# salute-developers/GigaAM

Hardware: AMD Instinct MI355X
Metric: RTFx v2_ctc batch32x20s (log-mel + encoder + greedy decode) (higher is better)
Workload: dtype f32 (GEMMs: 3-term split on fp16 MFMA, fp32 accumulate)

## Files before the change

### gigaam_amd/_lib.py

```python
from __future__ import annotations

import ctypes as C
import os
from typing import Optional

_HERE = os.path.dirname(os.path.abspath(__file__))
LIB_NAME = "libgigaam_hip.so"
LIB_PATH = os.path.join(_HERE, LIB_NAME)

SUBS_CONV2D, SUBS_CONV1D = 0, 1
ATT_ROTARY, ATT_REL_POS = 0, 1
NORM_BATCH, NORM_LAYER = 0, 1
HEAD_NONE, HEAD_CTC, HEAD_RNNT, HEAD_EMO = 0, 1, 2, 3
DTYPE_F32, DTYPE_F16, DTYPE_BF16, DTYPE_F64, DTYPE_I64 = 0, 1, 2, 3, 4
GEMM_F32, GEMM_F16X3, GEMM_F16 = 0, 1, 2
RS_U8, RS_I16, RS_I24, RS_I32, RS_F32, RS_MULAW, RS_ALAW = range(7)
RS_FORM_SINGLE, RS_FORM_TABLE, RS_FORM_ROWS = 0, 1, 2
PF_CLASSES = ["gemm", "conv2", "attn", "norm", "convmod", "stem", "frontend", "decode", "misc", "align_bt", "align_out"]


class GamConfig(C.Structure):
    _fields_ = [(n, C.c_int32) for n in (
        "sample_rate", "n_mels", "hop_length", "win_length", "n_fft", "center",
        "feat_in", "n_layers", "d_model", "subsampling", "subs_kernel_size", "subsampling_factor",
        "ff_expansion_factor", "self_attention_model", "n_heads", "pos_emb_max_len",
        "conv_norm_type", "conv_kernel_size",
        "head_type", "num_classes", "pred_hidden", "pred_rnn_layers", "joint_hidden",
    )]


_P = C.c_void_p


class GamLnOp(C.Structure):
    _fields_ = ([(n, _P) for n in ("x", "out1", "out2", "w1", "b1", "w2", "b2", "rcos", "rsin", "row_t", "rs", "part", "pbias", "presid",
                                   "xstore")]
                + [(n, C.c_int32) for n in ("mode", "rows", "d", "split1", "split2", "dk", "ta", "rope_rows", "nsplit")]
                + [("eps", C.c_float), ("palpha", C.c_float)])


SIGNATURES = {
    "gam_abi_version": (C.c_int, []),
    "gam_create": (C.c_int, [C.POINTER(GamConfig), C.c_int, C.POINTER(_P)]),
    "gam_destroy": (None, [_P]),
    "gam_set_weight": (C.c_int, [_P, C.c_char_p, _P, C.c_int, C.POINTER(C.c_int64), C.c_int]),
    "gam_finalize": (C.c_int, [_P]),
    "gam_feat_frames": (C.c_int64, [_P, C.c_int64]),
    "gam_enc_frames": (C.c_int64, [_P, C.c_int64]),
    "gam_frontend": (C.c_int, [_P, _P, _P, C.c_int, C.c_int64, _P, _P, _P]),
    "gam_encode": (C.c_int, [_P, _P, _P, C.c_int, C.c_int64, _P, _P, _P]),
    "gam_encode_ex": (C.c_int, [_P, _P, _P, C.c_int, C.c_int64, _P, _P, C.c_int, _P, _P]),
    "gam_encode_varlen": (C.c_int, [_P, _P, _P, C.POINTER(C.c_int64), C.c_int, C.c_int64, _P, _P, C.c_int, _P, _P]),
    "gam_last_encode_rows": (C.c_int, [_P, C.POINTER(C.c_int)]),
    "gam_ctc_head": (C.c_int, [_P, _P, C.c_int, C.c_int64, _P, _P]),
    "gam_ctc_greedy": (C.c_int, [_P, _P, _P, C.c_int, C.c_int64, _P, _P, _P, _P]),
    "gam_ctc_align": (C.c_int, [_P, _P, _P, C.c_int, C.c_int64, _P, _P, C.c_int, _P, _P, _P, _P, _P, _P, _P]),
    "gam_op_ctc_align": (C.c_int, [_P, _P, _P, C.c_int, C.c_int64, C.c_int, _P, _P, C.c_int, _P, _P, _P, _P, _P, _P, _P]),
    "gam_op_ctc_align_long": (C.c_int, [_P, _P, C.c_int64, C.c_int, _P, C.c_int, _P, _P, _P, _P, _P, _P, _P]),
    "gam_op_ctc_star_row": (C.c_int, [_P, _P, _P, C.c_int, C.c_int64, C.c_int, C.c_float, _P, _P]),
    "gam_ctc_align_star": (C.c_int, [_P, _P, _P, C.c_int, C.c_int64, _P, _P, C.c_int, C.c_float, _P, _P, _P, _P, _P, _P, _P]),
    "gam_op_ctc_align_star": (C.c_int, [_P, _P, _P, C.c_int, C.c_int64, C.c_int, _P, _P, _P, C.c_int, _P, _P, _P, _P, _P, _P, _P]),
    "gam_op_ctc_align_long_star": (C.c_int, [_P, _P, C.c_int64, C.c_int, _P, _P, C.c_int, _P, _P, _P, _P, _P, _P, _P]),
    "gam_op_ctc_stitch": (C.c_int, [_P, _P, _P, C.c_int, C.c_int64, C.c_int, _P, _P, _P, _P, C.c_int64, _P, _P]),
    "gam_op_ctc_greedy_long": (C.c_int, [_P, _P, C.c_int64, C.c_int, _P, _P, _P, _P]),
    "gam_set_ctc_align_workspace": (C.c_int, [_P, C.c_int64]),
    "gam_tune_ctc_align_long": (C.c_int, [C.c_int, C.c_int]),
    "gam_ctc_kws": (C.c_int, [_P, _P, _P, C.c_int, C.c_int64, C.c_int, _P, _P, _P, _P, _P, _P]),
    "gam_op_ctc_kws": (C.c_int, [_P, _P, _P, C.c_int, C.c_int64, C.c_int, C.c_int, _P, _P, _P, _P, _P, _P]),
    "gam_set_keywords": (C.c_int, [_P, _P, _P, C.c_int, _P]),
    "gam_ctc_kws_state_bytes": (C.c_int64, [_P]),
    "gam_op_ctc_kws_stream": (C.c_int, [_P, _P, C.c_int64, C.c_int, C.c_int64, C.c_int, _P, C.c_int, _P, _P, _P, _P, _P, _P, _P]),
    "gam_ctc_beam": (C.c_int, [_P, _P, _P, C.c_int, C.c_int64, C.c_int, _P, _P, _P, _P, _P, _P]),
    "gam_op_ctc_beam": (C.c_int, [_P, _P, _P, C.c_int, C.c_int64, C.c_int, C.c_int, _P, _P, _P, _P, _P, _P]),
    "gam_ctc_beam_stream_bytes": (C.c_int64, [_P, C.c_int, C.c_int64]),
    "gam_op_ctc_beam_stream": (C.c_int, [_P, _P, C.c_int64, C.c_int, C.c_int64, C.c_int, C.c_int, _P, C.c_int64, _P, _P, _P, _P, _P, _P, _P]),
    "gam_set_hotwords": (C.c_int, [_P, _P, _P, C.c_int, C.c_float]),
    "gam_set_lm": (C.c_int, [_P, _P, C.c_int, _P, C.c_int64, C.c_int, _P, C.c_int64, C.c_int, C.c_int, C.c_int, C.c_int, C.c_int,
                             C.c_float, C.c_float, C.c_float]),
    "gam_rnnt_greedy": (C.c_int, [_P, _P, _P, C.c_int, C.c_int64, C.c_int, _P, _P, _P, _P, _P, C.c_int, _P]),
    "gam_rnnt_encp": (C.c_int, [_P, _P, C.c_int, C.c_int64, _P, _P]),
    "gam_op_rnnt_greedy": (C.c_int, [_P, _P, _P, C.c_int, C.c_int64, C.c_int, _P, _P, _P, _P]),
    "gam_rnnt_greedy_stream_bytes": (C.c_int64, [_P]),
    "gam_op_rnnt_greedy_stream": (C.c_int, [_P, _P, C.c_int64, C.c_int64, C.c_int, C.c_int, _P, C.c_int64, _P, _P, C.c_int64, _P, _P, _P]),
    "gam_ctc_beam_nbest": (C.c_int, [_P, _P, _P, C.c_int, C.c_int64, C.c_int, C.c_int, _P, _P, _P, _P, _P, _P, _P]),
    "gam_op_ctc_beam_nbest": (C.c_int, [_P, _P, _P, C.c_int, C.c_int64, C.c_int, C.c_int, C.c_int, _P, _P, _P, _P, _P, _P, _P]),
    "gam_rnnt_beam_nbest": (C.c_int, [_P, _P, _P, C.c_int, C.c_int64, C.c_int, C.c_int, C.c_int, _P, _P, _P, _P, _P, _P, _P]),
    "gam_op_rnnt_beam_nbest": (C.c_int, [_P, _P, _P, C.c_int, C.c_int64, C.c_int, C.c_int, C.c_int, _P, _P, _P, _P, _P, _P, _P]),
    "gam_rnnt_beam": (C.c_int, [_P, _P, _P, C.c_int, C.c_int64, C.c_int, C.c_int, _P, _P, _P, _P, _P, _P]),
    "gam_op_rnnt_beam": (C.c_int, [_P, _P, _P, C.c_int, C.c_int64, C.c_int, C.c_int, _P, _P, _P, _P, _P, _P]),
    "gam_rnnt_align": (C.c_int, [_P, _P, _P, C.c_int, C.c_int64, _P, _P, C.c_int, _P, _P, _P, _P, _P]),
    "gam_op_rnnt_align": (C.c_int, [_P, _P, _P, C.c_int, C.c_int64, _P, _P, C.c_int, _P, _P, _P, _P, _P, _P]),
    "gam_op_rnnt_lattice_align": (C.c_int, [_P, _P, _P, C.c_int, C.c_int64, C.c_int, _P, _P, C.c_int, _P, _P, _P, _P, _P]),
    "gam_set_rnnt_align_workspace": (C.c_int, [_P, C.c_int64]),
    "gam_ctc_confidence": (C.c_int, [_P, _P, _P, C.c_int, C.c_int64, _P, _P, _P, C.c_int, C.c_int, C.c_int, _P, _P, _P, _P]),
    "gam_op_ctc_confidence": (C.c_int, [_P, _P, _P, C.c_int, C.c_int64, C.c_int, _P, _P, _P, C.c_int, C.c_int, C.c_int, _P, _P, _P, _P]),
    "gam_op_ctc_confidence_long": (C.c_int, [_P, _P, C.c_int64, C.c_int, _P, _P, _P, C.c_int, C.c_int, C.c_int, C.c_int, _P, _P, _P, _P]),
    "gam_rnnt_confidence": (C.c_int, [_P, _P, _P, C.c_int, C.c_int64, _P, _P, _P, C.c_int, C.c_int, _P, _P, _P]),
    "gam_op_rnnt_confidence": (C.c_int, [_P, _P, _P, C.c_int, C.c_int64, _P, _P, _P, C.c_int, C.c_int, _P, _P, _P]),
    "gam_emo_probs": (C.c_int, [_P, _P, _P, C.c_int, C.c_int64, _P, _P]),
    "gam_rnnt_predict": (C.c_int, [_P, _P, _P, _P, C.c_int, _P, _P, _P, _P]),
    "gam_rnnt_joint": (C.c_int, [_P, _P, _P, C.c_int, C.c_int, C.c_int, _P, _P]),
    "gam_set_gemm_mode": (C.c_int, [_P, C.c_int]),
    "gam_get_gemm_mode": (C.c_int, [_P]),
    "gam_set_rnnt_cluster": (C.c_int, [_P, C.c_int]),
    "gam_get_rnnt_cluster": (C.c_int, [_P]),
    "gam_rnnt_cluster_plan_info": (C.c_int, [C.c_int] * 8 + [C.POINTER(C.c_int32)]),
    "gam_rnnt_last_decode": (C.c_int, [_P, C.POINTER(C.c_int32)]),
    "gam_debug_buffer_hash": (C.c_int, [_P, C.c_int, C.POINTER(C.c_uint64), C.POINTER(C.c_int64)]),
    "gam_range_flag": (C.c_int, [_P, C.POINTER(C.c_int), _P]),
    "gam_range_flag_fetch": (C.c_int, [_P, _P, _P]),
    "gam_op_gemm": (C.c_int, [_P, _P, _P, _P, _P, C.c_int, C.c_int, C.c_int, C.c_int, _P]),
    "gam_op_gemm_ex": (C.c_int, [_P, _P, _P, _P, _P, C.c_float, _P, C.c_int, C.c_int, C.c_int, C.c_int, _P]),
    "gam_op_gemm_fmt": (C.c_int, [_P, _P, _P, _P, _P, C.c_float, _P, C.c_int64, C.c_int, C.c_int, C.c_int, C.c_int, C.c_int, C.c_int, _P]),
    "gam_op_attention": (C.c_int, [_P, _P, _P, _P, _P, _P, C.c_int, C.c_int, C.c_int, _P]),
    "gam_op_attention_ex": (C.c_int, [_P, _P, _P, _P, C.c_int64, _P, _P, _P, C.c_int, C.c_int, C.c_int, C.c_int, _P, _P, _P, _P]),
    "gam_op_layernorm": (C.c_int, [_P, C.POINTER(GamLnOp), _P]),
    "gam_op_convmod": (C.c_int, [_P, _P, _P, _P, _P, _P, _P, _P, _P, C.c_int, C.c_int, C.c_int, C.c_int, C.c_int, C.c_int, C.c_int, _P]),
    "gam_tune_sp": (C.c_int, [C.c_int, C.c_int, C.c_int]),
    "gam_plan_sp": (C.c_int, [C.c_int, C.c_int, C.c_int, C.c_int, C.POINTER(C.c_int), C.POINTER(C.c_int), C.POINTER(C.c_int)]),
    "gam_plan_sp_ex": (C.c_int, [C.c_int, C.c_int, C.c_int, C.c_int, C.POINTER(C.c_int), C.POINTER(C.c_int), C.POINTER(C.c_int), C.POINTER(C.c_int)]),
    "gam_tune_sp_stages": (C.c_int, [C.c_int]),
    "gam_resample_plan": (C.c_int, [C.c_int, C.c_int, C.POINTER(C.c_int), C.POINTER(C.c_int), C.POINTER(C.c_int)]),
    "gam_resample_tile": (C.c_int, [C.c_int, C.c_int, C.POINTER(C.c_int), C.POINTER(C.c_int)]),
    "gam_resample_table": (C.c_int, [C.c_int, C.c_int, _P, _P]),
    "gam_resample_out_len": (C.c_int64, [C.c_int, C.c_int, C.c_int64]),
    "gam_op_resample": (C.c_int, [_P, C.c_int, C.c_int, C.c_int, _P, C.c_int, C.c_int64, C.c_int, C.c_int, _P, _P, _P, C.c_int64, _P, _P]),
    "gam_profile_enable": (C.c_int, [_P, C.c_int]),
    "gam_profile_pause": (C.c_int, [_P, C.c_int]),
    "gam_profile_read": (C.c_int, [_P, C.c_int, C.POINTER(C.c_double), C.POINTER(C.c_int64), C.POINTER(C.c_double)]),
    "gam_profile_read_bytes": (C.c_int, [_P, C.c_int, C.POINTER(C.c_double)]),
    "gam_last_error": (C.c_char_p, [_P]),
    "gam_comm_unique_id": (C.c_int, [C.c_char_p]),
    "gam_comm_create": (C.c_int, [C.c_char_p, C.c_int, C.c_int, C.c_int, C.POINTER(_P)]),
    "gam_comm_world": (C.c_int, [_P]),
    "gam_gather_ids": (C.c_int, [_P, _P, _P, _P, _P, C.c_int, C.c_int, _P, _P, _P, _P, _P]),
    "gam_comm_last_error": (C.c_char_p, [_P]),
    "gam_comm_destroy": (None, [_P]),
}

_lib: Optional[C.CDLL] = None


class GigaAMHipError(RuntimeError):
    pass


def load_library(path: Optional[str] = None) -> C.CDLL:
    global _lib
    if _lib is not None and path is None:
        return _lib
    p = path or os.environ.get("GIGAAM_HIP_LIB", LIB_PATH)
    if not os.path.exists(p):
        raise GigaAMHipError(
            f"{p} not found: the HIP extension is not built. Run `python -c 'import __graft_entry__ as g; g.build()'` "
            "(hipcc --offload-arch=gfx950). There is no CPU fallback.")
    lib = C.CDLL(p)
    for name, (res, args) in SIGNATURES.items():
        fn = getattr(lib, name)
        fn.restype = res
        fn.argtypes = args
    if lib.gam_abi_version() != 1:
        raise GigaAMHipError("libgigaam_hip.so ABI version mismatch")
    if path is None:
        _lib = lib
    return lib
```

### gigaam_amd/csrc/gam_api.hip

```cpp
#include <hip/hip_runtime.h>

#include <algorithm>
#include <cmath>
#include <cstdarg>
#include <cstdio>
#include <cstring>
#include <map>
#include <string>
#include <vector>

#include "../../include/gigaam_hip.h"
#include "gam_align.h"
#include "gam_align_long.h"
#include "gam_kws.h"
#include "gam_attn.h"
#include "gam_beam.h"
#include "gam_beam_stream.h"
#include "gam_rnnt_beam.h"
#include "gam_attn16.h"
#include "gam_comm.h"
#include "gam_common.h"
#include "gam_convmod.h"
#include "gam_decode.h"
#include "gam_rnnt_stream.h"
// ... 215 lines not shown
    if (x < 0x33000000u) return (uint16_t)sign;
    const int e = (int)(x >> 23);
    uint32_t m = (x & 0x7fffffu) | 0x800000u;
    const int shift = 126 - e;
    const uint32_t rem = m & ((1u << shift) - 1u), half = 1u << (shift - 1);
    m >>= shift;
    if (rem > half || (rem == half && (m & 1u))) ++m;
    return (uint16_t)(sign | m);
  }
  const uint32_t e = (x >> 23) - 112u;
  uint32_t m = x & 0x7fffffu;
  uint32_t h = (e << 10) | (m >> 13);
  const uint32_t rem = m & 0x1fffu;
  if (rem > 0x1000u || (rem == 0x1000u && (h & 1u))) ++h;
  return (uint16_t)(sign | h);
}

float half_to_float(uint16_t x) {
  const uint32_t sign = (x >> 15) & 1, exp = (x >> 10) & 0x1f, man = x & 0x3ff;
  uint32_t f;
  if (exp == 0) {
    if (man == 0) f = sign << 31;
    else {
      int e = -1; uint32_t m = man;
      do { ++e; m <<= 1; } while (!(m & 0x400));
      f = (sign << 31) | ((uint32_t)(127 - 15 - e) << 23) | ((m & 0x3ff) << 13);
    }
  } else if (exp == 31) f = (sign << 31) | 0x7f800000u | (man << 13);
  else f = (sign << 31) | ((exp + 127 - 15) << 23) | (man << 13);
  float r; memcpy(&r, &f, 4); return r;
}

int make_split(gam_handle* h, const std::vector<float>& w, W16& out, int K = 0, int conv_taps = 0) {
  float mx = 0.f;
  for (float v : w) mx = std::max(mx, fabsf(v));
  int shift = 0;
  if (mx > 0.f && std::isfinite(mx)) shift = (int)floorf(log2f(256.0f / mx));
  shift = std::max(-24, std::min(24, shift));
  const float sc = ldexpf(1.0f, shift);
  std::vector<uint16_t> hi(w.size()), lo(w.size());
  for (size_t i = 0; i < w.size(); ++i) {
    const float v = w[i] * sc;
    const uint16_t hb = float_to_half_bits(v);
    hi[i] = hb;
    lo[i] = float_to_half_bits(v - half_to_float(hb));
  }
  out.inv = ldexpf(1.0f, -shift);
  std::vector<uint16_t> hp(hi);
  if (conv_taps > 0 && K > 0 && (K / conv_taps) % 64 == 0 && w.size() % (size_t)K == 0) {
    const size_t C = (size_t)K / conv_taps, cb64 = C / 64;
    for (size_t n = 0; n < w.size() / K; ++n)
      for (size_t cb = 0; cb < cb64; ++cb)
        for (size_t t = 0; t < (size_t)conv_taps; ++t)
          for (size_t j = 0; j < 64; ++j)
            hp[n * K + (cb * conv_taps + t) * 64 + j] = hi[n * K + t * C + cb * 64 + j];
  }
  out.h16 = (_Float16*)dev_upload(h, hp.data(), w.size() * 2, std::max<size_t>(w.size(), 8) * 2 + 64);
  if (!out.h16) return -2;
  if (K > 0 && K % 32 == 0 && w.size() % (size_t)K == 0) {
    std::vector<uint16_t> sp(w.size() * 2);
    for (size_t i = 0; i < w.size(); ++i) {
      const size_t n = i / K, k = i % K;
      size_t kb = k / 32;
      if (conv_taps > 0) {
        const size_t cblocks = (size_t)K / conv_taps / 32, t = kb / cblocks, cb = kb % cblocks;
        kb = cb * conv_taps + t;
      }
      const size_t o = n * 2 * (size_t)K + kb * 64 + (k % 32);
      sp[o] = hi[i];
      sp[o + 32] = lo[i];
    }
    out.sp = (_Float16*)dev_upload(h, sp.data(), sp.size() * 2, sp.size() * 2 + 64);
    if (!out.sp) return -2;
  }
  return 0;
}

const HostTensor* find(gam_handle* h, const std::string& key) {
  auto it = h->staged.find(key);
  return it == h->staged.end() ? nullptr : &it->second;
}

struct ProfScope {
  gam_handle* h;
  hipStream_t s;
  ProfEvent* ev = nullptr;
  ProfScope(gam_handle* h_, hipStream_t s_, int cls, double work) : h(h_), s(s_) {
    if (!h->prof_on || (h->prof_on == 2 && cls != GAM_PF_GEMM && cls != GAM_PF_CONV2)) return;
    if (h->prof_used == h->prof_events.size()) {
      ProfEvent e;
      if (hipEventCreate(&e.a) != hipSuccess || hipEventCreate(&e.b) != hipSuccess) return;
      h->prof_events.push_back(e);
    }
    ev = &h->prof_events[h->prof_used++];
    ev->cls = cls;
    h->prof_work[cls] += work;
    h->prof_launches[cls] += 1;
    hipEventRecord(ev->a, s);
  }
  ~ProfScope() {
    if (ev) hipEventRecord(ev->b, s);
  }
};

struct PendingReduce {
  const float* part = nullptr;
  int nsplit = 0;
  const float* bias = nullptr;
  const float* resid = nullptr;
  float alpha = 1.0f;
  GamGemmArgs full;
  int act = 0;
  void clear() { part = nullptr; nsplit = 0; }
};

int flush_pending(gam_handle* h, hipStream_t s, PendingReduce* p) {
  if (p == nullptr || p->part == nullptr) return 0;
  const hipError_t e = gam_launch_splitk_reduce(p->full, p->act, p->nsplit, s);
  const int M = p->full.M, N = p->full.N;
  p->clear();
  if (e != hipSuccess) return fail(h, -2, "split-K reduce launch (M=%d N=%d): %s", M, N, hipGetErrorString(e));
  return 0;
}

static inline bool split_mode(const gam_handle* h) { return h->gemm_mode != GAM_GEMM_F32; }

int gemm(gam_handle* h, hipStream_t s, const GamGemmArgs& a_in, int act, int cls = GAM_PF_GEMM, const W16* w16 = nullptr,
         PendingReduce* defer = nullptr) {
  GamGemmArgs a = a_in;
  if (int r = flush_pending(h, s, defer)) return r;
  a.range_flag = h->use_range ? h->range_flag : nullptr;
  if (!split_mode(h)) a.c_guard = 0;
  ProfScope ps(h, s, cls, 2.0 * (double)a.M * (double)a.N * (double)a.K);
  if (ps.ev) {
    const double abytes = a.a_mode == 0 ? ((double)(a.M - 1) * (double)std::min<long>(a.lda, a.K) + a.K) * 4.0
                                        : (double)a.M / a.conv_f2 * 2.0 * a.conv_fp * a.conv_c * 4.0;
    h->prof_bytes[cls] += abytes * (a.n_switch > 0 ? 2.0 : 1.0) + 4.0 * a.N * a.K + 4.0 * a.M * a.N * (a.R ? 2.0 : 1.0);
  }
  hipError_t e;
  if (a.Asp != nullptr) {
    if (!split_mode(h)) return fail(h, -2, "sp32 A operand outside the split-fp16 GEMM mode");
    if (w16 == nullptr || w16->sp == nullptr) return fail(h, -2, "sp32 A without sp32 W planes");
    a.wscale_inv = w16->inv;
    a.Wsp = w16->sp;
    a.h16 = 0;
    if (a.a_fmt == 2) {
      if (a.K % 64 != 0 || (a.a_mode == 0 ? a.lda % 64 != 0 : a.conv_c % 64 != 0) || w16->h16 == nullptr)
        return fail(h, -2, "GAM_GEMM_F16: K / row pitch of a GEMM operand is not a multiple of 64 (M=%d N=%d K=%d)", a.M, a.N, a.K);
      a.h16 = 1; a.K /= 2; a.lda /= 2; a.conv_c /= 2;
      a.Wsp = w16->h16;
    }
    GamSpPlan plan = gam_gemm_sp_plan(a.M, a.N, a.K, a.a_mode, h->ncu);
    if (!h->use_splitk) plan.s = 1;
    a.sp_mt = plan.mt; a.sp_nw = plan.nw; a.sp_ns = plan.ns;
    GamGemmArgs full = a;
    if (plan.s > 1) {
      if (int r = ensure(h, h->splitk_ws, (size_t)plan.s * a.M * a.N + 64)) return r;
      a.splitk = plan.s; a.partial = h->splitk_ws.p;
    }
    e = gam_launch_gemm_sp(a, act, s);
    if (e != hipSuccess) return fail(h, -2, "sp gemm launch (M=%d N=%d K=%d): %s", a.M, a.N, a.K, hipGetErrorString(e));
    if (plan.s > 1 && defer != nullptr && h->fuse_reduce && act == GAM_ACT_NONE && !a.c_split && !a.c_guard && a.lens == nullptr &&
        !a.remap && a.ldc == a.N && a.bias != nullptr && a.R != nullptr && a.ldr == a.N) {
      defer->part = a.partial; defer->nsplit = plan.s; defer->bias = a.bias; defer->resid = a.R; defer->alpha = a.alpha;
      defer->full = full; defer->full.partial = a.partial; defer->act = act;
    } else if (plan.s > 1) {
      full.partial = a.partial;
      e = gam_launch_splitk_reduce(full, act, plan.s, s);
      if (e != hipSuccess) return fail(h, -2, "split-K reduce launch (M=%d N=%d): %s", a.M, a.N, hipGetErrorString(e));
    }
    return 0;
  }
  if (a.a_rs != nullptr || a.c_split) return fail(h, -2, "row-scaled A or split C without sp32 operands (M=%d N=%d K=%d)", a.M, a.N, a.K);
  int S = 1;
  if (h->use_splitk && a.a_mode == 0 && a.K % 32 == 0) {
    const int tiles = gam_cdiv(a.M, 128) * gam_cdiv(a.N, 128), nk = a.K / 32, ncu = 256;
    if (tiles * 2 <= ncu && nk >= 4) {
      S = std::min(16, std::min(ncu / tiles, nk / 2));
      while (S > 1 && nk % S != 0) --S;
    }
  }
  GamGemmArgs full = a;
  if (S > 1) {
    DevBuf& ws = cls == GAM_PF_DECODE ? h->dec_splitk_ws : h->splitk_ws;
    if (int r = ensure(h, ws, (size_t)S * a.M * a.N + 64)) return r;
    a.splitk = S; a.ldw = a.K; a.K = a.K / S; a.partial = ws.p;
  }
  e = gam_launch_gemm(a, act, s);
  if (e != hipSuccess) return fail(h, -2, "gemm launch (M=%d N=%d K=%d): %s", a.M, a.N, a.K, hipGetErrorString(e));
  if (S > 1) {
    full.partial = a.partial;
    e = gam_launch_splitk_reduce(full, act, S, s);
    if (e != hipSuccess) return fail(h, -2, "split-K reduce launch (M=%d N=%d): %s", a.M, a.N, hipGetErrorString(e));
  }
  return 0;
}

GamGemmArgs gemm_args(const float* A, long lda, const float* W, const float* bias, float* C, long ldc, int M, int N, int K) {
  GamGemmArgs g;
  memset(&g, 0, sizeof g);
  g.A = A; g.W = W; g.bias = bias; g.C = C; g.R = nullptr;
  g.M = M; g.N = N; g.K = K; g.lda = lda; g.ldc = ldc; g.ldr = ldc; g.alpha = 1.0f;
  g.rpb = 1; g.fdiv = 1;
  return g;
}

int layernorm(gam_handle* h, hipStream_t s, GamLnArgs a, int mode, PendingReduce* pend = nullptr) {
  if (pend != nullptr && pend->part != nullptr) {
    const GamGemmArgs& g = pend->full;
    if (a.x == g.C && a.rows == g.M && a.d == g.N && g.ldc == g.N) {
      a.part = pend->part; a.nsplit = pend->nsplit; a.pbias = pend->bias; a.presid = pend->resid; a.palpha = pend->alpha;
      a.xstore = const_cast<float*>(a.x);
      pend->clear();
    } else if (int r = flush_pending(h, s, pend)) {
      return r;
    }
  }
  const double bytes = (double)a.rows * a.d * 4.0 * (mode == 0 ? 2.0 : 3.0);
  ProfScope ps(h, s, GAM_PF_NORM, bytes);
  hipError_t e = gam_launch_layernorm(a, mode, s);
  if (e != hipSuccess) return fail(h, -2, "layernorm launch: %s", hipGetErrorString(e));
  return 0;
}

int64_t half_up(int64_t l) { return l <= 0 ? 0 : (l + 1) / 2; }

struct DecodeScope {
  gam_handle* h;
  hipStream_t s;
  DecodeScope(gam_handle* h_, hipStream_t s_) : h(h_), s(s_) {
    if (h->dec_evt == nullptr && hipEventCreateWithFlags(&h->dec_evt, hipEventDisableTiming) != hipSuccess) { h->dec_evt = nullptr; (void)hipGetLastError(); }
    if (h->dec_evt != nullptr && h->dec_evt_set && h->dec_stream != s) (void)hipStreamWaitEvent(s, h->dec_evt, 0);
  }
  ~DecodeScope() {
    if (h->dec_evt != nullptr && hipEventRecord(h->dec_evt, s) == hipSuccess) { h->dec_stream = s; h->dec_evt_set = true; }
  }
};

#define GAM_DECODE_ENTRY(h, stream)      \
  hipStream_t s = (hipStream_t)(stream); \
  if (!(h)) return -1;                   \
  HIPCHK(h, hipSetDevice((h)->device));  \
  DecodeScope ds(h, s)

int head_check(gam_handle* h, int want, const char* who) {
  if (!h) return -1;
  if (who && !h->finalized) return fail(h, -1, "%s before gam_finalize", who);
  if (h->cfg.head_type != want || !h->has_head)
    return fail(h, -1, "model has no %s head", want == GAM_HEAD_CTC ? "CTC" : want == GAM_HEAD_RNNT ? "RNN-T" : "emotion");
  return 0;
}

template <class Args> void rnnt_pred_weights(const gam_handle* h, Args& a) {
  a.gate_tab = h->lstm_tab; a.whh_t = h->lstm_whh_t; a.wih_x = h->lstm_wih_x; a.whh_x = h->lstm_whh_x; a.bias_x = h->lstm_bias_x;
}
template <class Args> void rnnt_joint_weights(const gam_handle* h, Args& a) {
  a.wpred_t = h->jn_pred_t; a.bpred = h->jn_pred_b; a.wout = h->jn_out_w; a.bout = h->jn_out_b;
}

}

extern "C" {

int gam_abi_version(void) { return GAM_ABI_VERSION; }

const char* gam_last_error(const gam_handle* h) { return h ? h->err.c_str() : "null handle"; }

int gam_create(const gam_config* cfg, int device_id, gam_handle** out) {
  if (!cfg || !out) return -1;
  gam_handle* h = new gam_handle();
  h->cfg = *cfg;
  h->device = device_id;
  *out = h;
  if (const char* e = getenv("GAM_SPLITK")) h->use_splitk = atoi(e);
  if (const char* e = getenv("GAM_PACK")) h->use_pack = atoi(e);
  if (const char* e = getenv("GAM_FUSE_REDUCE")) h->fuse_reduce = atoi(e);
  if (const char* e = getenv("GAM_GRAPH")) h->use_graph = atoi(e);
  if (const char* e = getenv("GAM_GRAPH_MAX_ROWS")) h->graph_max_rows = atoi(e);
  if (const char* e = getenv("GAM_RNNT_CLUSTER")) h->rnnt_cluster = std::max(-1, std::min(8, atoi(e)));
  if (const char* e = getenv("GAM_RNNT_ALIGN_WS")) h->ra_ws_limit = (size_t)std::max(1ll, atoll(e));
  if (const char* e = getenv("GAM_CTC_ALIGN_WS")) h->al_ws_limit = (size_t)std::max(1ll, atoll(e));
  if (const char* e = getenv("GAM_RNNT_EXCLUSIVE")) h->rnnt_exclusive = atoi(e);
  if (const char* e = getenv("GAM_RNNT_COOP")) h->rnnt_coop = atoi(e);
  if (const char* e = getenv("GAM_RNNT_FORCE_TIMEOUT")) h->rnnt_force_timeout = atoi(e);
  if (const char* e = getenv("GAM_RNNT_NO_REPAIR")) h->rnnt_no_repair = atoi(e);
  {
    int n = 0;
    if (hipDeviceGetAttribute(&n, hipDeviceAttributeMultiprocessorCount, device_id) == hipSuccess && n > 0) h->ncu = n;
    int co = 0;
    if (hipDeviceGetAttribute(&co, hipDeviceAttributeCooperativeLaunch, device_id) != hipSuccess || co == 0) h->rnnt_coop = 0;
  }
  if (const char* e = getenv("GAM_ROWSCALE")) h->use_rowscale = atoi(e);
  if (const char* e = getenv("GAM_RANGE")) h->use_range = atoi(e);
  if (const char* e = getenv("GAM_GEMM_MODE"))
    h->gemm_mode = strcmp(e, "f32") == 0 ? GAM_GEMM_F32 : (strcmp(e, "f16") == 0 ? GAM_GEMM_F16 : GAM_GEMM_F16X3);
  const gam_config& c = h->cfg;
  if (c.d_model <= 0 || c.n_heads <= 0 || c.d_model % c.n_heads != 0)
    return fail(h, -1, "bad d_model/n_heads %d/%d", c.d_model, c.n_heads);
  if (c.d_model / c.n_heads != GAM_ATT_DK) return fail(h, -1, "head dim %d unsupported (kernels are built for %d)", c.d_model / c.n_heads, GAM_ATT_DK);
  if (c.d_model % 64 != 0 || c.d_model > 1024) return fail(h, -1, "d_model %d unsupported", c.d_model);
  if (c.subsampling_factor != 4) return fail(h, -1, "subsampling_factor %d unsupported", c.subsampling_factor);
  if (c.subsampling == GAM_SUBS_CONV2D && c.subs_kernel_size != 3) return fail(h, -1, "conv2d stem needs kernel 3");
  if (c.subsampling == GAM_SUBS_CONV1D && c.subs_kernel_size != 5) return fail(h, -1, "conv1d stem needs kernel 5");
  if (c.win_length != c.n_fft) return fail(h, -1, "win_length != n_fft unsupported");
  if (c.n_mels > 64 || c.n_mels != c.feat_in) return fail(h, -1, "n_mels %d / feat_in %d unsupported", c.n_mels, c.feat_in);
  if (c.head_type == GAM_HEAD_RNNT && (c.pred_rnn_layers < 1 || c.pred_rnn_layers > 4 || c.pred_hidden > GAM_RNNT_MAXH || c.joint_hidden > GAM_RNNT_MAXH || c.num_classes > GAM_RNNT_MAXV || c.joint_hidden % 16 != 0 || c.pred_hidden % 16 != 0))
    return fail(h, -1, "RNN-T head shape unsupported");
// ... 623 lines not shown

static int enc_stem(gam_handle* h, hipStream_t s, const EncPlan& p, const EncBufs& w, const float* feat) {
  if (int r = p.conv2d ? stem_conv2d(h, s, p, w, feat) : stem_conv1d(h, s, p, w, feat)) return r;
  if (p.packed) {
    ProfScope ps(h, s, GAM_PF_STEM, (double)p.NR * p.D * 8.0);
    hipLaunchKernelGGL(gam_gather_rows_kernel, dim3(std::min(4096, gam_cdiv(p.NR * (p.D / 4), 256))), dim3(256), 0, s, h->y.p, w.row_src, h->x.p, p.NR, p.D);
    HIPCHK(h, hipGetLastError());
  }
  return 0;
}

static int launch_attention(gam_handle* h, hipStream_t s, const float* q, const float* k, const float* v, long ldq, float* ctx, int ctx_split,
                            const int* lens, const int* cu, int B, int Ta, int Tv, int H, const float* pbuf, const float* pos_u,
                            const float* pos_v) {
  const int D = H * GAM_ATT_DK;
  GamAttnArgs at;
  memset(&at, 0, sizeof at);
  at.q = q; at.k = k; at.v = v; at.ctx = ctx; at.ctx_split = ctx_split; at.lens = lens; at.cu = cu;
  at.B = B; at.Ta = Ta; at.Tv = Tv; at.H = H; at.ldq = ldq; at.ldv = ldq; at.ldo = D;
  at.scale = 1.0f / sqrtf((float)GAM_ATT_DK);
  at.pbuf = pbuf; at.pos_u = pos_u; at.pos_v = pos_v; at.ldp = D;
  hipError_t e = gam_launch_attn_mode(at, GAM_ATT_DK, split_mode(h), s, h->gemm_mode == GAM_GEMM_F16 ? 1 : 3, h->ncu);
  if (e != hipSuccess) return fail(h, -2, "attention launch: %s", hipGetErrorString(e));
  return 0;
}

static hipError_t launch_convmod(gam_handle* h, hipStream_t s, const float* u, float* z, const float* dw_w, const float* dw_b, const float* n_scale,
                                 const float* n_shift, const int* lens, const int* cu, int B, int Ta, int Tv, int d, int ks, bool layer_norm,
                                 int z_split) {
  GamConvModArgs cm;
  memset(&cm, 0, sizeof cm);
  cm.u = u; cm.z = z; cm.dw_w = dw_w; cm.dw_b = dw_b; cm.n_scale = n_scale; cm.n_shift = n_shift;
  cm.lens = lens; cm.cu = cu; cm.B = B; cm.Ta = Ta; cm.Tv = Tv; cm.d = d; cm.ks = ks; cm.eps = 1e-5f;
  cm.z_split = z_split; cm.range_flag = h->use_range ? h->range_flag : nullptr;
  return gam_launch_convmod(cm, layer_norm, s);
}

static int norm_to_y(gam_handle* h, hipStream_t s, const EncCtx& c, const float* w, const float* b, PendingReduce* pend) {
  GamLnArgs a = c.ln;
  a.x = h->x.p; a.out1 = h->y.p; a.w1 = w; a.b1 = b;
  a.split1 = c.p.spf;
  return layernorm(h, s, a, 0, pend);
}

static int ffn_block(gam_handle* h, hipStream_t s, const EncCtx& c, const float* w1, const float* b1, const W16& s_w1, const float* w2,
                     const float* b2, const W16& s_w2, PendingReduce* pend) {
  const int D = c.p.D, DFF = c.p.DFF, NR = c.p.NR, spf = c.p.spf;
  GamGemmArgs g = gemm_args(h->y.p, D, w1, b1, h->hbuf.p, DFF, NR, DFF, D);
  gemm_formats(g, spf, c.w.rs, spf, 1);
  if (int r = gemm(h, s, g, GAM_ACT_SILU, GAM_PF_GEMM, &s_w1)) return r;
  GamGemmArgs g2 = gemm_args(h->hbuf.p, DFF, w2, b2, h->x.p, D, NR, D, DFF);
  g2.R = h->x.p; g2.ldr = D; g2.alpha = 0.5f;
  gemm_formats(g2, spf, nullptr, 0, 0);
  return gemm(h, s, g2, GAM_ACT_NONE, GAM_PF_GEMM, &s_w2, pend);
}

static int attn_block(gam_handle* h, hipStream_t s, const EncCtx& c, const LayerW& L, PendingReduce* pend) {
  const EncPlan& p = c.p;
  const int D = p.D, NR = p.NR, Tv = p.Tv, spf = p.spf;
  float* const rs = c.w.rs;
  GamLnArgs a = c.ln;
  a.x = h->x.p; a.out1 = h->y.p; a.out2 = h->yr.p; a.w1 = L.ln_att_w; a.b1 = L.ln_att_b;
  a.split1 = spf; a.split2 = spf;
  if (int r = layernorm(h, s, a, p.rel ? 0 : 1, pend)) return r;
  const bool one_launch = p.rel || (p.sp && (2 * D) % 256 == 0);
  if (one_launch) {
    GamGemmArgs gq = gemm_args(p.rel ? h->y.p : h->yr.p, D, L.wqkv, L.bqkv, h->qkv.p, 3 * D, NR, 3 * D, D);
    gemm_formats(gq, spf, rs, 0, 1);
    if (!p.rel) { gq.Asp2 = reinterpret_cast<const _Float16*>(h->y.p); gq.n_switch = 2 * D; }
    if (int r = gemm(h, s, gq, GAM_ACT_NONE, GAM_PF_GEMM, &L.s_wqkv)) return r;
  } else {
    GamGemmArgs gq = gemm_args(h->yr.p, D, L.wqkv, L.bqkv, h->qkv.p, 3 * D, NR, 2 * D, D);
    gemm_formats(gq, spf, rs, 0, 1);
    if (int r = gemm(h, s, gq, GAM_ACT_NONE, GAM_PF_GEMM, &L.s_wqkv)) return r;
    W16 wv16 = L.s_wqkv;
    const size_t off = (size_t)2 * D * D;
    wv16.h16 += off;
    if (wv16.sp) wv16.sp += 2 * off;
    GamGemmArgs gv = gemm_args(h->y.p, D, L.wqkv + off, L.bqkv + 2 * D, h->qkv.p + 2 * D, 3 * D, NR, D, D);
    gemm_formats(gv, spf, rs, 0, 1);
    if (int r = gemm(h, s, gv, GAM_ACT_NONE, GAM_PF_GEMM, &wv16)) return r;
  }
  if (p.rel) {
    const size_t pe0 = (size_t)(h->cfg.pos_emb_max_len - 1 - (Tv - 1)) * D;
    GamGemmArgs gp = gemm_args(h->rel_pe + pe0, D, L.wpos, nullptr, h->pbuf.p, D, 2 * Tv - 1, D, D);
    if (p.sp) { gp.Asp = reinterpret_cast<const _Float16*>(h->rel_pe_sp + pe0); gp.a_fmt = 1; }
    if (int r = gemm(h, s, gp, GAM_ACT_NONE, GAM_PF_GEMM, &L.s_wpos)) return r;
  }
  {
    ProfScope ps(h, s, GAM_PF_ATTN, 4.0 * (double)p.B * p.H * (double)Tv * Tv * p.dk);
    if (int r = launch_attention(h, s, h->qkv.p, h->qkv.p + D, h->qkv.p + 2 * D, 3 * D, h->ctx.p, spf, p.B > 1 ? c.w.len2 : nullptr, c.w.cu, p.B,
                                 p.packed ? p.Tmax : p.Ta, Tv, p.H, p.rel ? h->pbuf.p : nullptr, L.pos_u, L.pos_v))
      return r;
  }
  GamGemmArgs go = gemm_args(h->ctx.p, D, L.wo, L.bo, h->x.p, D, NR, D, D);
  go.R = h->x.p; go.ldr = D;
  gemm_formats(go, spf, nullptr, 0, 0);
  return gemm(h, s, go, GAM_ACT_NONE, GAM_PF_GEMM, &L.s_wo, pend);
}

static int conv_block(gam_handle* h, hipStream_t s, const EncCtx& c, const LayerW& L, PendingReduce* pend) {
  const EncPlan& p = c.p;
  const int D = p.D, NR = p.NR, ks = h->cfg.conv_kernel_size;
  if (int r = norm_to_y(h, s, c, L.ln_conv_w, L.ln_conv_b, pend)) return r;
  GamGemmArgs g1 = gemm_args(h->y.p, D, L.pw1_w, L.pw1_b, h->ubuf.p, 2 * D, NR, 2 * D, D);
  gemm_formats(g1, p.spf, c.w.rs, 0, 0);
  if (int r = gemm(h, s, g1, GAM_ACT_NONE, GAM_PF_GEMM, &L.s_pw1)) return r;
  {
    ProfScope ps(h, s, GAM_PF_CONVMOD, (double)NR * D * 3 * 4.0);
    hipError_t e = launch_convmod(h, s, h->ubuf.p, h->zbuf.p, L.dw_w, L.dw_b, L.cn_scale, L.cn_shift, c.w.len2, c.w.cu, p.B,
                                  p.packed ? p.Tmax : p.Ta, p.Tv, D, ks, h->cfg.conv_norm_type == GAM_NORM_LAYER, p.spf);
    if (e != hipSuccess) return fail(h, -2, "conv-module launch (k=%d): %s", ks, hipGetErrorString(e));
  }
  GamGemmArgs g2 = gemm_args(h->zbuf.p, D, L.pw2_w, L.pw2_b, h->x.p, D, NR, D, D);
  g2.R = h->x.p; g2.ldr = D;
  gemm_formats(g2, p.spf, nullptr, 0, 0);
  return gemm(h, s, g2, GAM_ACT_NONE, GAM_PF_GEMM, &L.s_pw2, pend);
}

static int norm_out_block(gam_handle* h, hipStream_t s, const EncCtx& c, const LayerW& L, const LayerW* next, PendingReduce* pend) {
  GamLnArgs a = c.ln;
  a.x = h->x.p; a.out1 = h->x.p; a.w1 = L.ln_out_w; a.b1 = L.ln_out_b;
  if (next != nullptr) {
    a.out2 = h->y.p; a.w2 = next->ln_ff1_w; a.b2 = next->ln_ff1_b;
    a.split2 = c.p.spf;
    return layernorm(h, s, a, 2, pend);
  }
  a.rs = nullptr;
  return layernorm(h, s, a, 0, pend);
}

static int run_layers(gam_handle* h, hipStream_t s, const EncCtx& c) {
  const int nl = c.p.nl;
  if (nl > 0)
    if (int r = norm_to_y(h, s, c, h->layers[0].ln_ff1_w, h->layers[0].ln_ff1_b, nullptr)) return r;
  PendingReduce pend;
  for (int li = 0; li < nl; ++li) {
    const LayerW& L = h->layers[li];
    if (int r = ffn_block(h, s, c, L.ff1_w1, L.ff1_b1, L.s_ff1_w1, L.ff1_w2, L.ff1_b2, L.s_ff1_w2, &pend)) return r;
    if (int r = attn_block(h, s, c, L, &pend)) return r;
    if (int r = conv_block(h, s, c, L, &pend)) return r;
    if (int r = norm_to_y(h, s, c, L.ln_ff2_w, L.ln_ff2_b, &pend)) return r;
    if (int r = ffn_block(h, s, c, L.ff2_w1, L.ff2_b1, L.s_ff2_w1, L.ff2_w2, L.ff2_b2, L.s_ff2_w2, &pend)) return r;
    if (int r = norm_out_block(h, s, c, L, li + 1 < nl ? &h->layers[li + 1] : nullptr, &pend)) return r;
  }
  return flush_pending(h, s, &pend);
}

static int replay_layers(gam_handle* h, hipStream_t s, const EncCtx& c, bool* replayed) {
  typedef gam_handle::GraphEntry Entry;
  const EncPlan& p = c.p;
  *replayed = false;
  if (!p.graph) return 0;
  const GamSpForce& frc = gam_sp_force();
  const std::vector<int> key = {p.B, p.Ta, p.Tv, p.nl, h->gemm_mode, (int)p.sp, h->use_splitk, h->fuse_reduce, frc.mt.load(), frc.nw.load(), frc.s.load(), frc.ns.load()};
  Entry& ge = h->graphs[key];
  if (ge.gen != h->ws_generation) {
    if (ge.exec) { hipGraphExecDestroy(ge.exec); --h->graph_count; }
    ge = Entry();
    ge.gen = h->ws_generation;
  }
  if (ge.exec == nullptr && ge.seen == Entry::SEEN_ONCE && h->graph_count >= 32) ge.seen = Entry::PLAIN_ONLY;
  if (ge.exec == nullptr && ge.seen == Entry::SEEN_ONCE) {
    hipGraph_t graph = nullptr;
    if (h->cap_stream == nullptr && hipStreamCreateWithFlags(&h->cap_stream, hipStreamNonBlocking) != hipSuccess)
      h->cap_stream = nullptr;
    if (h->cap_stream != nullptr && hipStreamBeginCapture(h->cap_stream, hipStreamCaptureModeRelaxed) == hipSuccess) {
      const int r = run_layers(h, h->cap_stream, c);
      const hipError_t e = hipStreamEndCapture(h->cap_stream, &graph);
      if (r == 0 && e == hipSuccess && graph != nullptr && h->ws_generation == ge.gen &&
          hipGraphInstantiate(&ge.exec, graph, nullptr, nullptr, 0) != hipSuccess)
        ge.exec = nullptr;
      if (graph) hipGraphDestroy(graph);
    }
    (void)hipGetLastError();
    if (ge.exec == nullptr) { ge.seen = Entry::PLAIN_ONLY; ++h->graph_captures_failed; }
    else ++h->graph_count;
  }
  if (ge.exec != nullptr) {
    HIPCHK(h, hipGraphLaunch(ge.exec, s));
    *replayed = true;
    ++h->graph_replays;
  } else if (ge.seen == Entry::UNSEEN) {
    ge.seen = Entry::SEEN_ONCE;
  }
  return 0;
}

static int enc_outputs(gam_handle* h, hipStream_t s, const EncPlan& p, const EncBufs& w, float* encoded, float* tokens_out, int32_t* enc_len) {
  const int B = p.B, Ta = p.Ta, Tv = p.Tv, D = p.D;
  ProfScope ps(h, s, GAM_PF_MISC, (double)B * Tv * D * 8.0);
  if (encoded && p.packed) {
    hipLaunchKernelGGL(gam_unpack_transpose_kernel, dim3(gam_cdiv(D, 32), gam_cdiv(Tv, 32), B), dim3(256), 0, s, h->x.p, w.cu, w.len2, encoded, Tv, D);
    HIPCHK(h, hipGetLastError());
  } else if (encoded) {
    hipError_t e = gam_launch_transpose(h->x.p, encoded, B, Tv, D, (size_t)Ta * D, D, (size_t)D * Tv, Tv, s);
    if (e != hipSuccess) return fail(h, -2, "transpose launch: %s", hipGetErrorString(e));
  }
  if (tokens_out && p.packed) {
    hipLaunchKernelGGL(gam_unpack_rows_kernel, dim3(std::min(4096, gam_cdiv(B * Tv * (D / 4), 256))), dim3(256), 0, s, h->x.p, w.cu, w.len2, tokens_out, B, Tv, D);
    HIPCHK(h, hipGetLastError());
  } else if (tokens_out)
    HIPCHK(h, hipMemcpy2DAsync(tokens_out, (size_t)Tv * D * 4, h->x.p, (size_t)Ta * D * 4, (size_t)Tv * D * 4, B, hipMemcpyDeviceToDevice, s));
  if (enc_len) HIPCHK(h, hipMemcpyAsync(enc_len, w.elen, (size_t)B * sizeof(int), hipMemcpyDeviceToDevice, s));
  return 0;
}

static int encode_impl(gam_handle* h, const float* feat, const int64_t* feat_len, int B, int64_t T, float* encoded,
                       int32_t* enc_len, int n_layers_run, float* tokens_out, hipStream_t s, const int64_t* feat_len_host = nullptr) {
  if (!h || !h->finalized) return fail(h, -1, "gam_encode before gam_finalize");
  if (!h->has_encoder) return fail(h, -1, "this handle was finalized without encoder weights");
  EncCtx c;
  if (int r = enc_plan(h, B, T, n_layers_run, feat_len_host, c.p)) return r;
  HIPCHK(h, hipSetDevice(h->device));
  h->last_rows = c.p.NR;
  h->last_rows_padded = c.p.N;
  if (int r = enc_workspace(h, c.p, c.w)) return r;
  c.ln = enc_ln_args(h, c.p, c.w);
  if (int r = enc_lengths(h, s, c.p, c.w, feat_len)) return r;
  if (int r = enc_stem(h, s, c.p, c.w, feat)) return r;
  bool replayed = false;
  if (int r = replay_layers(h, s, c, &replayed)) return r;
  if (!replayed)
    if (int r = run_layers(h, s, c)) return r;
  return enc_outputs(h, s, c.p, c.w, encoded, tokens_out, enc_len);
}

int gam_encode(gam_handle* h, const float* feat, const int64_t* feat_len, int B, int64_t T, float* encoded, int32_t* enc_len,
               void* stream) {
  return encode_impl(h, feat, feat_len, B, T, encoded, enc_len, -1, nullptr, (hipStream_t)stream);
}

int gam_encode_ex(gam_handle* h, const float* feat, const int64_t* feat_len, int B, int64_t T, float* encoded, int32_t* enc_len,
                  int n_layers_run, float* tokens_out, void* stream) {
  return encode_impl(h, feat, feat_len, B, T, encoded, enc_len, n_layers_run, tokens_out, (hipStream_t)stream);
}

int gam_encode_varlen(gam_handle* h, const float* feat, const int64_t* feat_len, const int64_t* feat_len_host, int B, int64_t T,
                      float* encoded, int32_t* enc_len, int n_layers_run, float* tokens_out, void* stream) {
  return encode_impl(h, feat, feat_len, B, T, encoded, enc_len, n_layers_run, tokens_out, (hipStream_t)stream, feat_len_host);
}

static int to_tokens(gam_handle* h, const float* encoded, int B, int64_t Tp, hipStream_t s) {
  const int D = h->cfg.d_model;
  if (int r = ensure(h, h->tok, (size_t)B * Tp * D)) return r;
  ProfScope ps(h, s, GAM_PF_DECODE, (double)B * Tp * D * 8.0);
  hipError_t e = gam_launch_transpose(encoded, h->tok.p, B, D, (int)Tp, (size_t)D * Tp, Tp, (size_t)Tp * D, D, s);
  if (e != hipSuccess) return fail(h, -2, "transpose launch: %s", hipGetErrorString(e));
  return 0;
}

static int ctc_logits(gam_handle* h, const float* encoded, int B, int64_t Tp, hipStream_t s) {
  if (B <= 0 || Tp <= 0) return fail(h, -1, "bad shape B=%d T'=%lld", B, (long long)Tp);
  HIPCHK(h, hipSetDevice(h->device));
  const int D = h->cfg.d_model, V = h->cfg.num_classes;
  if (int r = to_tokens(h, encoded, B, Tp, s)) return r;
  if (int r = ensure(h, h->logits, (size_t)B * Tp * V)) return r;
  GamGemmArgs g = gemm_args(h->tok.p, D, h->ctc_w, h->ctc_b, h->logits.p, V, (int)(B * Tp), V, D);
  return gemm(h, s, g, GAM_ACT_NONE, GAM_PF_DECODE);
}

static int rnnt_encp(gam_handle* h, const float* encoded, int B, int64_t Tp, hipStream_t s, float* out = nullptr) {
  const int D = h->cfg.d_model, JH = h->cfg.joint_hidden;
  if (int r = to_tokens(h, encoded, B, Tp, s)) return r;
  if (!out)
    if (int r = ensure(h, h->encp, (size_t)B * Tp * JH)) return r;
  GamGemmArgs g = gemm_args(h->tok.p, D, h->jn_enc_w, h->jn_enc_b, out ? out : h->encp.p, JH, (int)(B * Tp), JH, D);
  return gemm(h, s, g, GAM_ACT_NONE, GAM_PF_DECODE);
}

static int ctc_log_probs(gam_handle* h, const float* encoded, int B, int64_t Tp, float* out, hipStream_t s) {
  if (int r = ctc_logits(h, encoded, B, Tp, s)) return r;
  const int V = h->cfg.num_classes, rows = (int)(B * Tp);
  ProfScope ps(h, s, GAM_PF_DECODE, (double)rows * V * 8.0);
  hipLaunchKernelGGL(gam_log_softmax_kernel, dim3(gam_cdiv(rows, 4)), dim3(256), 0, s, h->logits.p, out ? out : h->logits.p, rows, V);
  HIPCHK(h, hipGetLastError());
  return 0;
}

int gam_ctc_head(gam_handle* h, const float* encoded, int B, int64_t Tp, float* log_probs, void* stream) {
  if (int r = head_check(h, GAM_HEAD_CTC, "CTC head")) return r;
  GAM_DECODE_ENTRY(h, stream);
  return ctc_log_probs(h, encoded, B, Tp, log_probs, s);
}

int gam_ctc_greedy(gam_handle* h, const float* encoded, const int32_t* enc_len, int B, int64_t Tp, int32_t* ids,
                   int32_t* frames, int32_t* counts, void* stream) {
  if (int r = head_check(h, GAM_HEAD_CTC, "CTC head")) return r;
  GAM_DECODE_ENTRY(h, stream);
  if (int r = ctc_logits(h, encoded, B, Tp, s)) return r;
  const int V = h->cfg.num_classes;
  const size_t sm = ((size_t)Tp + GAM_CTC_NT / 64 + 8) * sizeof(int);
  if (sm > 60 * 1024) return fail(h, -1, "T'=%lld too long for the CTC greedy kernel", (long long)Tp);
  ProfScope ps(h, s, GAM_PF_DECODE, (double)B * Tp * V * 4.0);
  hipLaunchKernelGGL(gam_ctc_greedy_kernel, dim3(B), dim3(GAM_CTC_NT), sm, s, h->logits.p, enc_len, (int)Tp, V, ids, frames, counts);
  HIPCHK(h, hipGetLastError());
  return 0;
}

static int ctc_align_launch(gam_handle* h, const float* lp, const int32_t* enc_len, int B, int64_t Tp, int V, const int32_t* targets,
                            const int32_t* target_len, int Umax, int32_t* frame_labels, int32_t* tok_first, int32_t* tok_last,
                            float* score, float* loglik, int32_t* status, hipStream_t s, const float* star = nullptr) {
  if (B <= 0 || Tp <= 0 || V < 2) return fail(h, -1, "CTC alignment: bad shape B=%d T'=%lld V=%d", B, (long long)Tp, V);
  if (Tp > GAM_ALIGN_MAX_T) return fail(h, -1, "CTC alignment: T'=%lld frames exceed the limit %d", (long long)Tp, GAM_ALIGN_MAX_T);
  if (Umax < 0 || Umax > GAM_ALIGN_MAX_U) return fail(h, -1, "CTC alignment: Umax=%d tokens outside [0, %d]", Umax, GAM_ALIGN_MAX_U);
  if (!lp || !enc_len || !target_len || !frame_labels || !score || !loglik || !status ||
      (Umax > 0 && (!targets || !tok_first || !tok_last)))
    return fail(h, -1, "CTC alignment: NULL buffer");
// ... 1327 lines not shown
  return launch_attention(h, (hipStream_t)stream, q, k, v, (long)ldq, ctx, 0, lens, cu, B, Ta, Tv, H, pbuf, pos_u, pos_v);
}

int gam_op_layernorm(gam_handle* h, const gam_ln_op* op, void* stream) {
  if (!h) return -1;
  if (!op) return fail(h, -1, "layernorm: null argument block");
  const gam_ln_op& o = *op;
  if (o.mode < 0 || o.mode > 2) return fail(h, -1, "layernorm: mode %d outside 0..2", o.mode);
  if (o.rows <= 0 || o.d <= 0) return fail(h, -1, "layernorm: bad shape rows %d d %d", o.rows, o.d);
  if (o.split1 < 0 || o.split1 > 2 || o.split2 < 0 || o.split2 > 2)
    return fail(h, -1, "layernorm: store format %d / %d outside 0..2", o.split1, o.split2);
  if (!o.out1 || !o.w1 || !o.b1) return fail(h, -1, "layernorm: out1 / w1 / b1 are mandatory");
  if (!o.part && !o.x) return fail(h, -1, "layernorm: x is mandatory without part");
  if (o.part && o.mode != 2 && !o.xstore) return fail(h, -1, "layernorm: part without xstore");
  if (o.mode != 0 && !o.out2) return fail(h, -1, "layernorm: mode %d needs out2", o.mode);
  if (o.mode == 2 && (!o.w2 || !o.b2)) return fail(h, -1, "layernorm: mode 2 needs w2 / b2");
  if (o.mode == 1) {
    if (!o.rcos || !o.rsin || o.rope_rows <= 0) return fail(h, -1, "layernorm: mode 1 needs rcos / rsin of rope_rows > 0 rows");
    if (o.dk <= 0) return fail(h, -1, "layernorm: mode 1 needs dk > 0");
    if (!o.row_t && o.ta <= 0) return fail(h, -1, "layernorm: mode 1 needs row_t or ta > 0");
  }
  auto al16 = [](const void* p) { return (reinterpret_cast<uintptr_t>(p) & 15) == 0; };
  if (!al16(o.x) || !al16(o.out1) || !al16(o.out2) || !al16(o.w1) || !al16(o.b1) || !al16(o.w2) || !al16(o.b2) || !al16(o.rcos) ||
      !al16(o.rsin) || !al16(o.part) || !al16(o.pbias) || !al16(o.presid) || !al16(o.xstore))
    return fail(h, -1, "layernorm: operands must be 16-byte aligned");
  HIPCHK(h, hipSetDevice(h->device));
  GamLnArgs a;
  memset(&a, 0, sizeof a);
  a.x = o.x; a.out1 = o.out1; a.out2 = o.out2; a.w1 = o.w1; a.b1 = o.b1; a.w2 = o.w2; a.b2 = o.b2;
  a.rcos = o.rcos; a.rsin = o.rsin; a.rows = o.rows; a.d = o.d; a.ta = o.ta; a.dk = o.dk; a.eps = o.eps;
  a.split1 = o.split1; a.split2 = o.split2; a.rs = o.rs; a.rope_rows = o.rope_rows;
  a.part = o.part; a.nsplit = o.nsplit; a.pbias = o.pbias; a.presid = o.presid; a.palpha = o.palpha; a.xstore = o.xstore;
  a.row_t = o.row_t;
  hipError_t e = gam_launch_layernorm(a, o.mode, (hipStream_t)stream);
  if (e != hipSuccess)
    return fail(h, -2, "layernorm launch (mode %d, rows %d, d %d, dk %d, split %d/%d, nsplit %d): %s", o.mode, o.rows, o.d, o.dk,
                o.split1, o.split2, o.part ? o.nsplit : 0, hipGetErrorString(e));
  return 0;
}

int gam_op_convmod(gam_handle* h, const float* u, float* z, const float* dw_w, const float* dw_b, const float* n_scale,
                   const float* n_shift, const int32_t* lens, const int32_t* cu, int B, int Ta, int Tv, int d, int ks, int layer_norm,
                   int z_split, void* stream) {
  if (!h) return -1;
  if (!h->finalized) return fail(h, -1, "gam_op_convmod before gam_finalize");
  if (!u || !z || !dw_w || !dw_b || !n_scale || !n_shift || !lens) return fail(h, -1, "conv module: null operand");
  if (B <= 0 || Ta <= 0 || Tv <= 0 || d <= 0) return fail(h, -1, "conv module: bad shape B %d Ta %d Tv %d d %d", B, Ta, Tv, d);
  if (cu == nullptr && Tv > Ta) return fail(h, -1, "conv module: Tv %d > Ta %d in the padded layout", Tv, Ta);
  if (z_split < 0 || z_split > 2) return fail(h, -1, "conv module: store format %d outside 0..2", z_split);
  if (z_split && d % 32 != 0) return fail(h, -1, "conv module: a split-fp16 z needs d %% 32 == 0 (d = %d)", d);
  auto al16 = [](const void* p) { return (reinterpret_cast<uintptr_t>(p) & 15) == 0; };
  if (d % 4 == 0 && (!al16(u) || !al16(z) || !al16(dw_b) || !al16(n_scale) || !al16(n_shift)))
    return fail(h, -1, "conv module: operands must be 16-byte aligned");
  HIPCHK(h, hipSetDevice(h->device));
  hipError_t e = launch_convmod(h, (hipStream_t)stream, u, z, dw_w, dw_b, n_scale, n_shift, lens, cu, B, Ta, Tv, d, ks, layer_norm != 0, z_split);
  if (e != hipSuccess) return fail(h, -2, "conv-module launch (k=%d, d=%d, %s): %s", ks, d, layer_norm ? "LayerNorm" : "BatchNorm", hipGetErrorString(e));
  return 0;
}

int gam_set_gemm_mode(gam_handle* h, int mode) {
  if (!h || (mode != GAM_GEMM_F32 && mode != GAM_GEMM_F16X3 && mode != GAM_GEMM_F16)) return fail(h, -1, "unknown GEMM mode %d", mode);
  h->gemm_mode = mode;
  return 0;
}

int gam_get_gemm_mode(const gam_handle* h) { return h ? h->gemm_mode : -1; }

int gam_debug_buffer_hash(gam_handle* h, int which, uint64_t* hash_out, int64_t* floats_out) {
  if (!h || !hash_out) return -1;
  const DevBuf* b = which == 0 ? &h->tok : which == 1 ? &h->encp : which == 2 ? &h->rnnt_x : which == 3 ? &h->logits : nullptr;
  if (!b) return fail(h, -1, "no such buffer %d", which);
  HIPCHK(h, hipSetDevice(h->device));
  HIPCHK(h, hipDeviceSynchronize());
  std::vector<uint32_t> host(b->cap);
  if (b->cap) HIPCHK(h, hipMemcpy(host.data(), b->p, b->cap * sizeof(float), hipMemcpyDeviceToHost));
  uint64_t x = 1469598103934665603ull;
  for (uint32_t v : host) { x ^= v; x *= 1099511628211ull; }
  *hash_out = x;
  if (floats_out) *floats_out = (int64_t)b->cap;
  return 0;
}

int gam_set_rnnt_cluster(gam_handle* h, int workgroups_per_utterance) {
  if (!h) return -1;
  if (workgroups_per_utterance < -1 || workgroups_per_utterance > 8) return fail(h, -1, "cluster size %d outside -1 (auto) .. 8", workgroups_per_utterance);
  h->rnnt_cluster = workgroups_per_utterance;
  return 0;
}

int gam_get_rnnt_cluster(gam_handle* h) { return h ? h->rnnt_cluster : -2; }

int gam_rnnt_cluster_plan_info(int ncu, int cluster, int exclusive, int B, int H, int JH, int V, int L, int32_t* out) {
  if (!out || B <= 0 || H <= 0 || JH <= 0 || V <= 0 || L <= 0) return -1;
  const RnntClusterPlan p = rnnt_cluster_plan(ncu, cluster, exclusive, B, H, JH, V, L);
  memset(out, 0, 8 * sizeof(int32_t));
  if (p.C == 0) return 0;
  out[0] = p.C; out[1] = p.nr; out[2] = p.kern; out[3] = p.resident ? 1 : 0;
  out[4] = p.wout_slice_in_lds; out[5] = p.wpred_slice_in_lds; out[6] = (int32_t)p.lds; out[7] = (int32_t)p.grid;
  return 0;
}

int gam_rnnt_last_decode(gam_handle* h, int32_t* out) {
  if (!h || !out) return -1;
  out[0] = h->last_rnnt_c; out[1] = h->last_rnnt_kern; out[2] = h->last_rnnt_refused;
  return 0;
}

int gam_last_encode_rows(gam_handle* h, int* rows_padded) {
  if (!h) return -1;
  if (rows_padded) *rows_padded = h->last_rows_padded;
  return h->last_rows;
}

int gam_range_flag(gam_handle* h, int* flag_host, void* stream) {
  if (!h || !flag_host) return -1;
  if (!h->finalized) return fail(h, -1, "gam_range_flag before gam_finalize");
  HIPCHK(h, hipSetDevice(h->device));
  hipStream_t s = (hipStream_t)stream;
  HIPCHK(h, hipMemcpyAsync(flag_host, h->range_flag, sizeof(int), hipMemcpyDeviceToHost, s));
  HIPCHK(h, hipMemsetAsync(h->range_flag, 0, sizeof(int), s));
  HIPCHK(h, hipStreamSynchronize(s));
  return 0;
}

int gam_range_flag_fetch(gam_handle* h, int32_t* flag_dev, void* stream) {
  if (!h || !flag_dev) return -1;
  if (!h->finalized) return fail(h, -1, "gam_range_flag_fetch before gam_finalize");
  HIPCHK(h, hipSetDevice(h->device));
  hipStream_t s = (hipStream_t)stream;
  HIPCHK(h, hipMemcpyAsync(flag_dev, h->range_flag, sizeof(int), hipMemcpyDeviceToDevice, s));
  HIPCHK(h, hipMemsetAsync(h->range_flag, 0, sizeof(int), s));
  return 0;
}

int gam_plan_sp(int M, int N, int K, int n_cu, int* mt, int* nw, int* splitk) {
  if (M <= 0 || N <= 0 || K <= 0 || K % 32 != 0 || !mt || !nw || !splitk) return -1;
  const GamSpPlan p = gam_gemm_sp_plan(M, N, K, 0, n_cu > 0 ? n_cu : 256);
  *mt = p.mt; *nw = p.nw; *splitk = p.s;
  return 0;
}

int gam_tune_sp(int mt, int nw, int splitk) {
  GamSpForce& f = gam_sp_force();
  f.mt = mt; f.nw = nw; f.s = splitk;
  return 0;
}

int gam_tune_sp_stages(int stages) {
  if (stages != 0 && stages != 2 && stages != 3) return -1;
  gam_sp_force().ns = stages;
  return 0;
}

int gam_plan_sp_ex(int M, int N, int K, int n_cu, int* mt, int* nw, int* splitk, int* stages) {
  if (M <= 0 || N <= 0 || K <= 0 || K % 32 != 0 || !mt || !nw || !splitk || !stages) return -1;
  const GamSpPlan p = gam_gemm_sp_plan(M, N, K, 0, n_cu > 0 ? n_cu : 256);
  *mt = p.mt; *nw = p.nw; *splitk = p.s; *stages = p.ns;
  return 0;
}

int gam_resample_plan(int rate_in, int rate_out, int* up, int* down, int* taps) {
  GamRsPlan p;
  const int rc = gam_rs_plan(rate_in, rate_out, &p);
  if (rc != 0) return rc;
  if (up) *up = (int)p.N;
  if (down) *down = (int)p.O;
  if (taps) *taps = p.K;
  return 0;
}

int gam_resample_tile(int rate_in, int rate_out, int* tile, int* form) {
  GamRsPlan p;
  const int rc = gam_rs_plan(rate_in, rate_out, &p);
  if (rc != 0) return rc;
  if (tile) *tile = p.tile;
  if (form) *form = p.form;
  return 0;
}

int gam_resample_table(int rate_in, int rate_out, float* coeff, int32_t* first) {
  GamRsPlan p;
  const int rc = gam_rs_plan(rate_in, rate_out, &p);
  if (rc != 0) return rc;
  if (!coeff || !first) return -1;
  gam_rs_table(p, coeff, first);
  return 0;
}

int64_t gam_resample_out_len(int rate_in, int rate_out, int64_t n_in) {
  GamRsPlan p;
  if (gam_rs_plan(rate_in, rate_out, &p) != 0) return -1;
  return gam_rs_out_len(p, n_in);
}

int gam_op_resample(const void* src, int fmt, int channels, int channel, const int64_t* len_in, int B, int64_t frames, int rate_in, int rate_out,
                    const float* coeff, const int32_t* first, float* dst, int64_t L_out, int64_t* len_out, void* stream) {
  return gam_rs_run(src, fmt, channels, channel, len_in, B, frames, rate_in, rate_out, coeff, first, dst, L_out, len_out, (hipStream_t)stream);
}

int gam_profile_enable(gam_handle* h, int on) {
  if (!h) return -1;
  h->prof_on = on;
  h->prof_used = 0;
  for (int i = 0; i < GAM_PF_NCLASS; ++i) { h->prof_work[i] = 0; h->prof_launches[i] = 0; h->prof_bytes[i] = 0; }
  return 0;
}

int gam_profile_pause(gam_handle* h, int on) {
  if (!h) return -1;
  h->prof_on = on;
  return 0;
}

int gam_profile_read_bytes(gam_handle* h, int cls, double* bytes) {
  if (!h || cls < 0 || cls >= GAM_PF_NCLASS || !bytes) return -1;
  *bytes = h->prof_bytes[cls];
  return 0;
}

int gam_profile_read(gam_handle* h, int cls, double* ms, int64_t* launches, double* work) {
  if (!h || cls < 0 || cls >= GAM_PF_NCLASS) return -1;
  double tot = 0;
  for (size_t i = 0; i < h->prof_used; ++i) {
    ProfEvent& e = h->prof_events[i];
    if (e.cls != cls) continue;
    HIPCHK(h, hipEventSynchronize(e.b));
    float t = 0;
    HIPCHK(h, hipEventElapsedTime(&t, e.a, e.b));
    tot += t;
  }
  if (ms) *ms = tot;
  if (launches) *launches = h->prof_launches[cls];
  if (work) *work = h->prof_work[cls];
  return 0;
}

}
```

### gigaam_amd/csrc/gam_gemm.h

```cpp
#pragma once
#include "gam_common.h"
#include <stdlib.h>

struct GamGemmArgs {
  const float* A;
  const float* W;
  const float* bias;
  const float* R;
  float* C;
  int M, N, K;
  long lda, ldc, ldr;
  float alpha;
  int a_mode;
  int conv_fp;
  int conv_c;
  int conv_f2;
  const int* lens;
  int rpb, fdiv;
  int remap, out_rpb, out_shift, rows_valid;
  int skip_pad;
  const _Float16* Asp;
  const _Float16* Wsp;
  const _Float16* Asp2;
  int n_switch;
  int c_split;
  int splitk;
  long ldw;
  float* partial;
  int sp_mt, sp_nw;
  int sp_ns;
  int a_fmt;
  int h16;
  int ntiles;
  float wscale_inv;
  const float* a_rs;
  int* range_flag;
  int c_guard;
  long long* tlog;
};

#define GAM_GEMM_BM 128
#define GAM_GEMM_BN 128
#define GAM_GEMM_BK 32
#define GAM_GEMM_LD 36
#define GAM_GEMM_SMEM ((GAM_GEMM_BM + GAM_GEMM_BN) * GAM_GEMM_LD * 4)

template <int ACT>
__device__ __forceinline__ void gam_gemm_epilogue(const GamGemmArgs& g, const f32x16& acc00, const f32x16& acc01,
                                                  const f32x16& acc10, const f32x16& acc11, int m0, int n0, int wm,
                                                  int wn, int lane) {
  const int lcol = lane & 31;
  const int lrow4 = 4 * (lane >> 5);
  if (g.partial != nullptr) {
    float* P = g.partial + (size_t)blockIdx.y * (size_t)g.M * (size_t)g.N;
#pragma unroll
    for (int tm = 0; tm < 2; ++tm)
#pragma unroll
      for (int r = 0; r < 16; ++r) {
        const int row = m0 + wm * 64 + tm * 32 + (r & 3) + 8 * (r >> 2) + lrow4;
        if (row >= g.M) continue;
#pragma unroll
        for (int tn = 0; tn < 2; ++tn) {
          const int col = n0 + wn * 64 + tn * 32 + lcol;
          if (col < g.N)
            P[(size_t)row * g.N + col] = tm == 0 ? (tn == 0 ? acc00[r] : acc01[r]) : (tn == 0 ? acc10[r] : acc11[r]);
        }
      }
    return;
  }
#pragma unroll
  for (int tm = 0; tm < 2; ++tm) {
#pragma unroll
    for (int r = 0; r < 16; ++r) {
      const int row = m0 + wm * 64 + tm * 32 + (r & 3) + 8 * (r >> 2) + lrow4;
      if (row >= g.M) continue;
      bool masked = false;
      long orow = row;
      if (g.lens != nullptr || g.remap) {
        const int bb = row / g.rpb, tt = row - bb * g.rpb;
        if (g.lens != nullptr) masked = (tt / g.fdiv) >= g.lens[bb];
        if (g.remap) {
          if (tt >= g.rows_valid) continue;
          orow = (long)bb * g.out_rpb + tt + g.out_shift;
        }
      }
#pragma unroll
      for (int tn = 0; tn < 2; ++tn) {
        const int col = n0 + wn * 64 + tn * 32 + lcol;
        if (col >= g.N) continue;
        float v = tm == 0 ? (tn == 0 ? acc00[r] : acc01[r]) : (tn == 0 ? acc10[r] : acc11[r]);
        if (g.bias != nullptr) v += g.bias[col];
        if (ACT == GAM_ACT_SILU) v = gam_silu(v);
        if (ACT == GAM_ACT_RELU) v = fmaxf(v, 0.0f);
        if (masked) v = 0.0f;
        v *= g.alpha;
        if (g.R != nullptr) v += g.R[orow * g.ldr + col];
        if (g.c_guard) gam_range_note(g.range_flag, v, 0.f, 0.f, 0.f);
        g.C[orow * g.ldc + col] = v;
      }
    }
  }
}

template <int ACT>
__global__ __launch_bounds__(256, 3) void gam_gemm_f32_kernel(GamGemmArgs g) {
  extern __shared__ __attribute__((aligned(16))) float gam_smem[];
  if (g.splitk > 1) { const size_t ko = (size_t)blockIdx.y * (size_t)g.K; g.A += ko; g.W += ko; }
  constexpr int BM = GAM_GEMM_BM, BN = GAM_GEMM_BN, BK = GAM_GEMM_BK, LD = GAM_GEMM_LD;
  float* As = gam_smem;
  float* Bs = gam_smem + BM * LD;

  const int tid = threadIdx.x;
  const int lane = tid & 63;
  const int wave = __builtin_amdgcn_readfirstlane(tid >> 6);
  const int wm = wave >> 1, wn = wave & 1;

  const int nbn = (g.N + BN - 1) / BN;
  const int total = gridDim.x;
  const int bid = blockIdx.x;
  const int q8 = total >> 3, r8 = total & 7;
  const int xcd = bid & 7;
  const int lid = (xcd < r8 ? xcd * (q8 + 1) : r8 * (q8 + 1) + (xcd - r8) * q8) + (bid >> 3);
  const int m0 = (lid / nbn) * BM;
  const int n0 = (lid % nbn) * BN;

  const int lrow = tid >> 3;
  const int lc4 = (tid & 7) * 4;
  auto a_row_off = [&](int i) -> size_t {
    int m = m0 + lrow + 32 * i;
    m = m < g.M ? m : g.M - 1;
    if (g.a_mode == 0) return (size_t)m * (size_t)g.lda;
    const int fr = m / g.conv_f2, f = m - fr * g.conv_f2;
    return ((size_t)fr * 2 * g.conv_fp + 2 * f) * (size_t)g.conv_c;
  };
  auto w_row_off = [&](int i) -> size_t {
    int n = n0 + lrow + 32 * i;
    n = n < g.N ? n : g.N - 1;
    return (size_t)n * (size_t)g.ldw;
  };
  const float* pa0 = g.A + a_row_off(0) + lc4;
  const float* pa1 = g.A + a_row_off(1) + lc4;
  const float* pa2 = g.A + a_row_off(2) + lc4;
  const float* pa3 = g.A + a_row_off(3) + lc4;
  const float* pw0 = g.W + w_row_off(0) + lc4;
  const float* pw1 = g.W + w_row_off(1) + lc4;
  const float* pw2 = g.W + w_row_off(2) + lc4;
  const float* pw3 = g.W + w_row_off(3) + lc4;

  f32x16 acc00, acc01, acc10, acc11;
#pragma unroll
  for (int r = 0; r < 16; ++r) { acc00[r] = 0.f; acc01[r] = 0.f; acc10[r] = 0.f; acc11[r] = 0.f; }

  const int nkf = g.K / BK;
  const int nk = (g.K + BK - 1) / BK;
  float4 va0, va1, va2, va3, vb0, vb1, vb2, vb3;

#define GAM_GLOAD(KT)                                                           \
  {                                                                             \
    const int k0_ = (KT) * BK;                                                  \
    size_t ka_ = (size_t)k0_;                                                   \
    if (g.a_mode != 0) {                                                        \
      const int tap_ = k0_ / g.conv_c, c0_ = k0_ - tap_ * g.conv_c;             \
      const int kh_ = tap_ / 3, kw_ = tap_ - kh_ * 3;                           \
      ka_ = ((size_t)kh_ * g.conv_fp + kw_) * (size_t)g.conv_c + c0_;           \
    }                                                                           \
    va0 = *reinterpret_cast<const float4*>(pa0 + ka_);                          \
    va1 = *reinterpret_cast<const float4*>(pa1 + ka_);                          \
    va2 = *reinterpret_cast<const float4*>(pa2 + ka_);                          \
    va3 = *reinterpret_cast<const float4*>(pa3 + ka_);                          \
    vb0 = *reinterpret_cast<const float4*>(pw0 + k0_);                          \
    vb1 = *reinterpret_cast<const float4*>(pw1 + k0_);                          \
    vb2 = *reinterpret_cast<const float4*>(pw2 + k0_);                          \
    vb3 = *reinterpret_cast<const float4*>(pw3 + k0_);                          \
  }
#define GAM_GLOAD_TAIL(KT)                                                      \
  {                                                                             \
    const int k0_ = (KT) * BK;                                                  \
    const bool in_ = k0_ + lc4 < g.K;                                           \
    const int ko_ = in_ ? k0_ : k0_ - lc4;                                      \
    const float4 z_ = make_float4(0.f, 0.f, 0.f, 0.f);                          \
    va0 = *reinterpret_cast<const float4*>(pa0 + ko_);                          \
    va1 = *reinterpret_cast<const float4*>(pa1 + ko_);                          \
    va2 = *reinterpret_cast<const float4*>(pa2 + ko_);                          \
    va3 = *reinterpret_cast<const float4*>(pa3 + ko_);                          \
    vb0 = *reinterpret_cast<const float4*>(pw0 + ko_);                          \
    vb1 = *reinterpret_cast<const float4*>(pw1 + ko_);                          \
    vb2 = *reinterpret_cast<const float4*>(pw2 + ko_);                          \
    vb3 = *reinterpret_cast<const float4*>(pw3 + ko_);                          \
    if (!in_) { va0 = z_; va1 = z_; va2 = z_; va3 = z_; vb0 = z_; vb1 = z_; vb2 = z_; vb3 = z_; } \
  }
// ... 137 lines not shown
```

### gigaam_amd/csrc/gam_gemm_sp.h

```cpp
#pragma once
#include "gam_gemm.h"
#include <type_traits>
#if defined(GAM_SP_INSTRUMENT) && GAM_SP_INSTRUMENT
#include <algorithm>
#include <vector>
#endif

#ifndef GAM_SP_INSTRUMENT
#define GAM_SP_INSTRUMENT 0
#endif
#if GAM_SP_INSTRUMENT
#define GAM_SP_TL(i)                                                                  \
  if (g.tlog != nullptr && threadIdx.x == 0) {                                        \
    g.tlog[(size_t)lid * 8 + (i)] = wall_clock64();                                   \
    if ((i) == 1 || (i) == 2) g.tlog[(size_t)lid * 8 + 4 + (i)] = clock64();          \
    if ((i) == 0) g.tlog[(size_t)lid * 8 + 7] = blockIdx.x;                            \
  }
#else
#define GAM_SP_TL(i)
#endif

template <int MT, int NW, int NS = 2>
struct GamGemmSpCfg {
  static constexpr int BM = 64 * MT;
  static constexpr int BN = 64 * NW;
  static constexpr int NWAVES = 2 * NW;
  static constexpr int NT = 64 * NWAVES;
  static constexpr int A_BYTES = BM * 128;
  static constexpr int W_BYTES = BN * 128;
  static constexpr int STAGE = A_BYTES + W_BYTES;
  static constexpr int SMEM = NS * STAGE;
  static constexpr int NAI = BM / 8 / NWAVES;
  static constexpr int NWI = BN / 8 / NWAVES;
};

__device__ __forceinline__ int gam_sp_key(int row) { return ((row >> 1) & 7) ^ ((row >> 3) & 2); }

enum : int {
  GAM_EPI_SP32 = 1,
  GAM_EPI_F16 = 2,
  GAM_EPI_CFMT = 3,
  GAM_EPI_RESID = 4,
  GAM_EPI_ALPHA = 8,
  GAM_EPI_ROWS = 16,
  GAM_EPI_GUARD = 32,
  GAM_EPI_TAIL = 64,
  GAM_EPI_PART = 128,
  GAM_EPI_GENERIC = 256
};

template <int ACT, int EPI, int MT, int NW, int NS = 2, bool H16 = false>
__global__ __launch_bounds__(128 * NW, NW == 2 ? 2 : 1) void gam_gemm_sp_kernel(GamGemmArgs g) {
  extern __shared__ __attribute__((aligned(16))) unsigned char gam_smem_sp[];
  using Cfg = GamGemmSpCfg<MT, NW, NS>;
  constexpr int BM = Cfg::BM, BN = Cfg::BN, NAI = Cfg::NAI, NWI = Cfg::NWI, NWAVES = Cfg::NWAVES;
  typedef __attribute__((address_space(3))) void* lds_ptr_t;
  typedef const __attribute__((address_space(1))) void* glb_ptr_t;

  const int tid = threadIdx.x;
  const int lane = tid & 63;
  const int wave = __builtin_amdgcn_readfirstlane(tid >> 6);
  const int wm = wave / NW, wn = wave % NW;

  const int nbn = (g.N + BN - 1) / BN;
  const int total = gridDim.x;
  const int q8 = total >> 3, r8 = total & 7;
  const int bid = blockIdx.x;
  const int xcd = bid & 7;
  const int lid = (xcd < r8 ? xcd * (q8 + 1) : r8 * (q8 + 1) + (xcd - r8) * q8) + (bid >> 3);
  int tm = lid / nbn, tn = lid % nbn;
  if (g.skip_pad) {
    tm = bid / nbn;
    tn = bid % nbn;
  }
  const int m0 = tm * BM;
  const int n0 = tn * BN;
  if (g.skip_pad && g.lens != nullptr) {
    const int mlast = m0 + BM - 1 < g.M ? m0 + BM - 1 : g.M - 1;
    const int b0 = m0 / g.rpb;
    if (b0 == mlast / g.rpb && (m0 - b0 * g.rpb) / g.fdiv >= g.lens[b0]) return;
  }
  GAM_SP_TL(0);

  auto a_row_off = [&](int m) -> size_t {
    m = m < g.M ? m : g.M - 1;
    if (g.a_mode == 0) return (size_t)m * (size_t)g.lda;
    const int fr = m / g.conv_f2, ff = m - fr * g.conv_f2;
    return ((size_t)fr * 2 * g.conv_fp + 2 * ff) * (size_t)g.conv_c;
  };
  const size_t a_tile0 = a_row_off(m0);
  const unsigned char* Ab = reinterpret_cast<const unsigned char*>(g.n_switch > 0 && n0 >= g.n_switch ? g.Asp2 : g.Asp) + a_tile0 * 4;
  const unsigned char* Wb = reinterpret_cast<const unsigned char*>(g.Wsp) + (size_t)n0 * (size_t)g.K * 4;
  unsigned a_src[NAI], w_src[NWI];
#pragma unroll
  for (int i = 0; i < NAI; ++i) {
    const int row = 8 * (wave + NWAVES * i) + (lane >> 3);
    const int slot = (lane & 7) ^ gam_sp_key(row);
    a_src[i] = (unsigned)((a_row_off(m0 + row) - a_tile0) * 4) + slot * 16;
  }
#pragma unroll
  for (int i = 0; i < NWI; ++i) {
    const int row = 8 * (wave + NWAVES * i) + (lane >> 3);
    const int slot = (lane & 7) ^ gam_sp_key(row);
    int n = n0 + row;
    n = n < g.N ? n : g.N - 1;
    w_src[i] = (unsigned)(n - n0) * (unsigned)g.K * 4u + slot * 16;
  }

  f32x4 acc[2 * MT][4];
#pragma unroll
  for (int i = 0; i < 2 * MT; ++i)
#pragma unroll
    for (int j = 0; j < 4; ++j)
#pragma unroll
      for (int r = 0; r < 4; ++r) acc[i][j][r] = 0.f;

  const int nslice = g.splitk > 1 ? g.splitk : 1;
  const int nk = g.K / 32 / nslice;
  const int kt_first = (nslice > 1 ? (int)blockIdx.y : 0) * nk, kt_end = kt_first + nk;
  int d_kt = kt_first, d_c0 = 0, d_kw = 0, d_kh = 0;
  if (g.a_mode != 0) {
    const int cb = kt_first / 9, t9 = kt_first - cb * 9;
    d_c0 = 32 * cb; d_kh = t9 / 3; d_kw = t9 - d_kh * 3;
  }
  auto dma_ka = [&]() -> size_t {
    if (g.a_mode == 0) return (size_t)d_kt * 128;
    return (((size_t)d_kh * g.conv_fp + d_kw) * (size_t)g.conv_c + d_c0) * 4;
  };
  auto dma_advance = [&]() {
    if (d_kt + 1 >= kt_end) return;
    ++d_kt;
    if (g.a_mode == 0) return;
    if (++d_kw == 3) {
      d_kw = 0;
      if (++d_kh == 3) { d_kh = 0; d_c0 += 32; }
    }
  };
  auto issue = [&](int stage) {
    unsigned char* sb = gam_smem_sp + stage * Cfg::STAGE + wave * 1024;
    const unsigned char* ab = Ab + dma_ka();
    const unsigned char* wb = Wb + (size_t)d_kt * 128;
#pragma unroll
    for (int i = 0; i < NAI; ++i)
      __builtin_amdgcn_global_load_lds((glb_ptr_t)(ab + a_src[i]), (lds_ptr_t)(sb + i * (NWAVES * 1024)), 16, 0, 0);
#pragma unroll
    for (int i = 0; i < NWI; ++i)
      __builtin_amdgcn_global_load_lds((glb_ptr_t)(wb + w_src[i]), (lds_ptr_t)(sb + Cfg::A_BYTES + i * (NWAVES * 1024)), 16, 0, 0);
    dma_advance();
  };

  const int fi = lane & 15, fg = lane >> 4;
  const int wr = 8 * (fi >> 2) + (fi & 3);
  int o_a[2][2], o_w[2][2];
#pragma unroll
  for (int pl = 0; pl < 2; ++pl)
#pragma unroll
    for (int x = 0; x < 2; ++x) {
      o_a[pl][x] = fi * 128 + (((4 * pl + fg) ^ gam_sp_key(fi + 16 * x)) << 4);
      o_w[pl][x] = (wr + 4 * x) * 128 + (((4 * pl + fg) ^ gam_sp_key(wr + 4 * x)) << 4);
    }
  const int a_base = wm * (BM / 2) * 128;
  const int w_base = Cfg::A_BYTES + wn * 64 * 128;

  gam_half8 fah[2 * MT], fal[2 * MT], fwh[4], fwl[4];
  constexpr int NTERM = H16 ? 2 : 3;
  constexpr int QM = 2 * NTERM * MT;
  constexpr int NG = NAI + NWI;
  constexpr int G3 = QM - 2 * MT;
  static_assert(4 + 2 * MT <= QM && G3 + QM - 4 >= NG, "quadrant too short for its reads + DMA pieces");
#define GAM_SPLD(P) (*reinterpret_cast<const gam_half8*>(P))
#define GAM_SP_RDW(NH, Q, ST)                                                                     \
  {                                                                                               \
    const int q_ = (Q);                                                                           \
    if (q_ < 2) fwh[2 * (NH) + (q_ & 1)] = GAM_SPLD((ST) + w_base + (NH) * 4096 + o_w[0][q_ & 1]);  \
    else fwl[2 * (NH) + (q_ & 1)] = GAM_SPLD((ST) + w_base + (NH) * 4096 + o_w[1][q_ & 1]);         \
  }
#define GAM_SP_RDA(MH, Q, ST)                                                                     \
  {                                                                                               \
    const int q_ = (Q), i_ = (MH) * MT + q_ % MT;                                                 \
    if (q_ < MT) fah[i_] = GAM_SPLD((ST) + a_base + i_ * 2048 + o_a[0][i_ & 1]);                  \
    else fal[i_] = GAM_SPLD((ST) + a_base + i_ * 2048 + o_a[1][i_ & 1]);                          \
  }
#define GAM_SP_MFMA(MH, NH, T)                                                                    \
  {                                                                                               \
    const int term_ = (T) / (2 * MT), i_ = (MH) * MT + ((T) % (2 * MT)) / 2, j_ = 2 * (NH) + ((T) & 1); \
     \
    acc[i_][j_] = __builtin_amdgcn_mfma_f32_16x16x32_f16(term_ == 1 ? fwl[j_] : fwh[j_],          \
                                                         (H16 ? term_ == 1 : term_ == 2) ? fal[i_] : fah[i_], acc[i_][j_], 0, 0, 0); \
  }
  auto half0 = [&](const unsigned char* st) {
#pragma unroll
    for (int t = 0; t < QM; ++t) {
      GAM_SP_MFMA(0, 0, t);
      if (t < 4) GAM_SP_RDW(1, t, st)
      else if (t < 4 + 2 * MT) GAM_SP_RDA(1, t - 4, st)
      __builtin_amdgcn_sched_barrier(0);
    }
#pragma unroll
    for (int t = 0; t < QM; ++t) {
      GAM_SP_MFMA(0, 1, t);
      __builtin_amdgcn_sched_barrier(0);
    }
  };
  auto half1 = [&](const unsigned char* sn, int istage) {
    const unsigned char* ab = Ab + dma_ka();
    const unsigned char* wb = Wb + (size_t)d_kt * 128;
    unsigned char* sb = gam_smem_sp + istage * Cfg::STAGE + wave * 1024;
    dma_advance();
#pragma unroll
    for (int u = 0; u < 2 * QM; ++u) {
      if (u < QM) {
        GAM_SP_MFMA(1, 0, u);
        if (u < 2 * MT) GAM_SP_RDA(0, u, sn)
      } else {
        GAM_SP_MFMA(1, 1, u - QM);
        if (u - QM < 4) GAM_SP_RDW(0, u - QM, sn)
      }
      const int gi = u < QM ? u - 2 * MT : (u - QM < 4 ? -1 : G3 + u - QM - 4);
      if (gi >= 0 && gi < NG) {
        if (gi < NAI)
          __builtin_amdgcn_global_load_lds((glb_ptr_t)(ab + a_src[gi % NAI]), (lds_ptr_t)(sb + gi * (NWAVES * 1024)), 16, 0, 0);
        else
          __builtin_amdgcn_global_load_lds((glb_ptr_t)(wb + w_src[(gi - NAI + NWI) % NWI]),
                                           (lds_ptr_t)(sb + Cfg::A_BYTES + (gi - NAI) * (NWAVES * 1024)), 16, 0, 0);
      }
      __builtin_amdgcn_sched_barrier(0);
    }
  };

  constexpr int VMW = (NS - 2) * NG;
  static_assert(VMW < 64, "vmcnt field");
#pragma unroll
  for (int st_ = 0; st_ < NS; ++st_) issue(st_);
  if constexpr (NS == 2) {
    __builtin_amdgcn_s_waitcnt(0x0070);
    __syncthreads();
  } else {
    asm volatile("s_waitcnt vmcnt(%0) lgkmcnt(0)\n\ts_barrier" ::"n"(VMW) : "memory");
  }
  GAM_SP_TL(1);
#pragma unroll
  for (int q = 0; q < 2 * MT; ++q) GAM_SP_RDA(0, q, gam_smem_sp);
#pragma unroll
  for (int q = 0; q < 4; ++q) GAM_SP_RDW(0, q, gam_smem_sp);
  int s_cur = 0;
  for (int kt = 0; kt < nk; ++kt) {
    const int s_nxt = s_cur + 1 == NS ? 0 : s_cur + 1;
    const unsigned char* st = gam_smem_sp + s_cur * Cfg::STAGE;
    const unsigned char* sn = gam_smem_sp + s_nxt * Cfg::STAGE;
    half0(st);
    if constexpr (NS == 2) {
      __builtin_amdgcn_s_waitcnt(0x0070);
      __syncthreads();
    } else {
      asm volatile("s_waitcnt vmcnt(%0) lgkmcnt(0)\n\ts_barrier" ::"n"(VMW) : "memory");
    }
    half1(sn, s_cur);
    s_cur = s_nxt;
  }
#undef GAM_SPLD
#undef GAM_SP_RDW
#undef GAM_SP_RDA
#undef GAM_SP_MFMA
  __builtin_amdgcn_s_waitcnt(0x0070);
  GAM_SP_TL(2);

  const int mw = m0 + wm * (BM / 2), nw = n0 + wn * 64;

  constexpr bool GEN = (EPI & GAM_EPI_GENERIC) != 0;
  const bool part = GEN ? g.partial != nullptr : (EPI & GAM_EPI_PART) != 0;
  const int cfmt = GEN ? g.c_split : (EPI & GAM_EPI_CFMT);
  const bool resid = !part && (GEN ? g.R != nullptr : (EPI & GAM_EPI_RESID) != 0);
  const bool scaled = GEN || (EPI & GAM_EPI_ALPHA) != 0;
  const bool need_bt = !part && (GEN ? (g.lens != nullptr || g.remap) : (EPI & GAM_EPI_ROWS) != 0);
  const bool guard = GEN ? (g.c_guard && g.range_flag != nullptr) : (EPI & GAM_EPI_GUARD) != 0;
  const bool tail = GEN ? (g.N & 4) != 0 : (EPI & GAM_EPI_TAIL) != 0;
  const int lrow = lane & 15, lq8 = (lane >> 4) * 8;
  const float accscale = g.wscale_inv;
  const int ecol0 = nw + lq8;
  bool c_ok[2], c_both[2];
#pragma unroll
  for (int pp = 0; pp < 2; ++pp) {
    c_ok[pp] = ecol0 + 32 * pp < g.N;
    c_both[pp] = !tail || ecol0 + 32 * pp + 4 < g.N;
  }
  f32x4 bv[2][2];
#pragma unroll
  for (int pp = 0; pp < 2; ++pp)
#pragma unroll
    for (int hf = 0; hf < 2; ++hf) {
      const int col = ecol0 + 32 * pp + 4 * hf;
      bv[pp][hf] = (g.bias != nullptr && col < g.N) ? *reinterpret_cast<const f32x4*>(g.bias + col) : (f32x4){0.f, 0.f, 0.f, 0.f};
    }
  const long c_col = cfmt == 1 ? 2L * ((ecol0 >> 5) * 64 + (ecol0 & 31)) : (cfmt == 2 ? 2L * ecol0 : 4L * ecol0);
  const long c_pitch = cfmt == 2 ? 2 * g.ldc : 4 * g.ldc;
  const int c_step = cfmt == 2 ? 64 : 128;
  unsigned char* const c_base = reinterpret_cast<unsigned char*>(g.C) + c_col;
  bool r_ok[2 * MT], r_masked[2 * MT];
  long r_orow[2 * MT];
  float r_rsc[2 * MT];
  int bb = 0, tt = 0;
  if (need_bt) { bb = (mw + lrow) / g.rpb; tt = (mw + lrow) - bb * g.rpb; }
#pragma unroll
  for (int i = 0; i < 2 * MT; ++i) {
    const int row = mw + 16 * i + lrow;
    bool ok = row < g.M, masked = false;
    long orow = row;
    if (need_bt) {
      if (i > 0) {
        tt += 16;
        if (g.rpb < 16) { bb = row / g.rpb; tt = row - bb * g.rpb; }
        else if (tt >= g.rpb) { tt -= g.rpb; ++bb; }
      }
      if (ok) {
        if (g.lens != nullptr) masked = tt >= g.lens[bb] * g.fdiv;
        if (g.remap) {
          if (tt >= g.rows_valid) ok = false;
          orow = (long)bb * g.out_rpb + tt + g.out_shift;
        }
      }
    }
    r_rsc[i] = accscale * ((ok && g.a_rs != nullptr) ? g.a_rs[row] : 1.0f);
    r_ok[i] = ok; r_masked[i] = masked; r_orow[i] = orow;
  }
  if (part) {
#pragma unroll
    for (int i = 0; i < 2 * MT; ++i) {
      if (!r_ok[i]) continue;
      float* P = g.partial + ((size_t)blockIdx.y * (size_t)g.M + (size_t)(mw + 16 * i + lrow)) * (size_t)g.N + ecol0;
#pragma unroll
      for (int pp = 0; pp < 2; ++pp)
#pragma unroll
        for (int hf = 0; hf < 2; ++hf)
          if (ecol0 + 32 * pp + 4 * hf < g.N) *reinterpret_cast<f32x4*>(P + 32 * pp + 4 * hf) = acc[i][2 * pp + hf] * r_rsc[i];
    }
  }
#define GAM_SP_LDR(I, D)                                                                          \
  {                                                                                               \
    const float* rrow_ = g.R + r_orow[I] * g.ldr + ecol0;                                         \
    _Pragma("unroll") for (int pp = 0; pp < 2; ++pp) _Pragma("unroll") for (int hf = 0; hf < 2; ++hf)  \
      D[pp][hf] = (r_ok[I] && ecol0 + 32 * pp + 4 * hf < g.N) ? *reinterpret_cast<const f32x4*>(rrow_ + 32 * pp + 4 * hf)  \
                                                             : (f32x4){0.f, 0.f, 0.f, 0.f};       \
  }
  f32x4 rv[2][2], rn[2][2];
  float gmax = 0.f;
  if (resid) GAM_SP_LDR(0, rv);
#pragma unroll
  for (int i = 0; i < 2 * MT; ++i) {
    if (resid && i + 1 < 2 * MT) GAM_SP_LDR(i + 1, rn);
    const bool masked = r_masked[i];
    const float rsc = r_rsc[i];
    if (r_ok[i] && !part) {
      unsigned char* const crow = c_base + r_orow[i] * c_pitch;
#pragma unroll
      for (int pp = 0; pp < 2; ++pp) {
        if (!c_ok[pp]) continue;
        const bool both = c_both[pp];
        f32x4 v[2];
#pragma unroll
        for (int hf = 0; hf < 2; ++hf) {
          f32x4 t = acc[i][2 * pp + hf];
          t = t * rsc + bv[pp][hf];
          if (ACT == GAM_ACT_SILU) { t.x = gam_silu(t.x); t.y = gam_silu(t.y); t.z = gam_silu(t.z); t.w = gam_silu(t.w); }
          if (ACT == GAM_ACT_RELU) { t.x = fmaxf(t.x, 0.f); t.y = fmaxf(t.y, 0.f); t.z = fmaxf(t.z, 0.f); t.w = fmaxf(t.w, 0.f); }
          if (need_bt && masked) t = (f32x4){0.f, 0.f, 0.f, 0.f};
          if (scaled) t = t * g.alpha;
          if (resid) t += rv[pp][hf];
          if (tail && !both && hf == 1) t = (f32x4){0.f, 0.f, 0.f, 0.f};
          v[hf] = t;
        }
        if (guard) {
          gmax = fmaxf(gmax, fmaxf(fmaxf(fabsf(v[0].x), fabsf(v[0].y)), fmaxf(fabsf(v[0].z), fabsf(v[0].w))));
          gmax = fmaxf(gmax, fmaxf(fmaxf(fabsf(v[1].x), fabsf(v[1].y)), fmaxf(fabsf(v[1].z), fabsf(v[1].w))));
        }
        unsigned char* const cp = crow + pp * c_step;
        if (cfmt == 2) {
          const gam_half4 h0 = __builtin_convertvector(v[0], gam_half4), h1 = __builtin_convertvector(v[1], gam_half4);
          if (both) *reinterpret_cast<gam_half8*>(cp) = (gam_half8){h0[0], h0[1], h0[2], h0[3], h1[0], h1[1], h1[2], h1[3]};
          else *reinterpret_cast<gam_half4*>(cp) = h0;
        } else if (cfmt) {
          gam_half4 hi0, lo0, hi1, lo1;
          gam_split4(v[0], hi0, lo0);
          gam_split4(v[1], hi1, lo1);
          if (both) {
            *reinterpret_cast<gam_half8*>(cp) = (gam_half8){hi0[0], hi0[1], hi0[2], hi0[3], hi1[0], hi1[1], hi1[2], hi1[3]};
            *reinterpret_cast<gam_half8*>(cp + 64) = (gam_half8){lo0[0], lo0[1], lo0[2], lo0[3], lo1[0], lo1[1], lo1[2], lo1[3]};
          } else {
            *reinterpret_cast<gam_half4*>(cp) = hi0;
            *reinterpret_cast<gam_half4*>(cp + 64) = lo0;
          }
        } else {
          *reinterpret_cast<f32x4*>(cp) = v[0];
          if (both) *reinterpret_cast<f32x4*>(cp + 16) = v[1];
        }
      }
    }
    if (resid && i + 1 < 2 * MT) {
#pragma unroll
      for (int pp = 0; pp < 2; ++pp)
#pragma unroll
        for (int hf = 0; hf < 2; ++hf) rv[pp][hf] = rn[pp][hf];
    }
  }
  if (guard && gmax > GAM_F16_SAFE_MAX) atomicOr(g.range_flag, 1);
#undef GAM_SP_LDR
#if GAM_SP_INSTRUMENT
  if (g.tlog != nullptr) { __builtin_amdgcn_s_waitcnt(0x0070); __syncthreads(); }
  GAM_SP_TL(3);
#endif
}

static inline bool gam_gemm_sp_epilogue_ok(const GamGemmArgs& a) {
  auto al16 = [](const void* p) { return (reinterpret_cast<uintptr_t>(p) & 15) == 0; };
  return a.N % 4 == 0 && a.ldc % 4 == 0 && al16(a.C) && (a.bias == nullptr || al16(a.bias)) &&
         (a.R == nullptr || (a.ldr % 4 == 0 && al16(a.R)));
}

template <int ACT, int EPI, int MT, int NW, int NS = 2, bool H16 = false>
static inline void gam_launch_gemm_sp_t(const GamGemmArgs& a, int grid, hipStream_t stream) {
  static std::atomic<unsigned long long> attr_devs{0};
  constexpr int smem = GamGemmSpCfg<MT, NW, NS>::SMEM;
  static_assert(smem <= 160 * 1024, "LDS stages do not fit a CU");
  auto kern = gam_gemm_sp_kernel<ACT, EPI, MT, NW, NS, H16>;
  if (gam_set_max_lds(reinterpret_cast<const void*>(kern), smem, attr_devs) != hipSuccess) return;
  hipLaunchKernelGGL(kern, dim3(grid, a.splitk > 1 ? a.splitk : 1), dim3(128 * NW), smem, stream, a);
}

static inline int gam_sp_epi_bits(const GamGemmArgs& a) {
  if (a.partial != nullptr) return GAM_EPI_PART;
  return (a.c_split & GAM_EPI_CFMT) | (a.R != nullptr ? GAM_EPI_RESID : 0) | (a.alpha != 1.0f ? GAM_EPI_ALPHA : 0) |
         ((a.lens != nullptr || a.remap) ? GAM_EPI_ROWS : 0) | ((a.c_guard && a.range_flag != nullptr) ? GAM_EPI_GUARD : 0) |
         ((a.N & 7) == 4 ? GAM_EPI_TAIL : 0);
}

struct GamSpPlan { int mt, nw, s, ns; };
struct GamSpForce {
  std::atomic<int> mt{0}, nw{0}, s{0}, ns{0};
  GamSpForce() {
    const char* e0 = getenv("GAM_SP_MT"); const char* e1 = getenv("GAM_SP_NW"); const char* e2 = getenv("GAM_SP_SPLITK");
    const char* e3 = getenv("GAM_SP_STAGES");
    mt = e0 ? atoi(e0) : 0; nw = e1 ? atoi(e1) : 0; s = e2 ? atoi(e2) : 0; ns = e3 ? atoi(e3) : 0;
  }
};
static inline bool gam_sp_has_ns3(int mt, int nw) { return (nw == 2 && (mt == 2 || mt == 3)) || (nw == 4 && mt == 2); }
static inline GamSpForce& gam_sp_force() { static GamSpForce f; return f; }
static inline double gam_gemm_sp_model(int M, int N, int K, int a_mode, int t, int w, int S, int ncu, int ns = 2) {
  const long wgs = (long)gam_cdiv(M, 64 * t) * gam_cdiv(N, 64 * w) * S;
  const int nkt = K / 32 / S;
  double t_kt, t_fix, rounds;
  if (ns == 3) {
    if (w == 4) { t_kt = 0.953; t_fix = S > 1 ? 6.62 : 12.8; }
    else { t_kt = 0.229 * t + 0.115; t_fix = S > 1 ? 4.76 : 12.0; }
    rounds = (double)((wgs + ncu - 1) / ncu);
  } else if (w == 4) {
    t_kt = 0.335 * t + 0.425;
    t_fix = S > 1 ? 6.2 : 13.2;
    rounds = (double)((wgs + ncu - 1) / ncu);
  } else {
    const bool shared = wgs > ncu;
    const double tk_u = 0.256 * t + 0.142, tf_u = S > 1 ? 4.9 : 14.1;
    t_kt = tk_u * (shared ? 1.82 : 1.0);
    t_fix = tf_u * (shared ? 0.73 : 1.0);
    rounds = (double)((wgs + (shared ? 2 : 1) * ncu - 1) / ((shared ? 2 : 1) * ncu));
    const long cap2 = 2L * ncu, rem = wgs % cap2;
    if (shared && wgs > cap2 && rem != 0 && rem <= ncu) {
      (void)a_mode;
      double us2 = (double)(wgs / cap2) * (nkt * t_kt + t_fix) + (nkt * tk_u + tf_u);
      if (S > 1) us2 += 7.1 + (double)(S + 2) * M * N * 4.0 / 3.87e6;
      return us2;
    }
  }
  (void)a_mode;
  double us = rounds * (nkt * t_kt + t_fix);
  if (S > 1) us += 7.1 + (double)(S + 2) * M * N * 4.0 / 3.87e6;
  return us;
}
static inline GamSpPlan gam_gemm_sp_plan(int M, int N, int K, int a_mode = 0, int ncu = 256) {
  GamSpForce& frc = gam_sp_force();
  const int f_mt = frc.mt.load(std::memory_order_relaxed), f_nw = frc.nw.load(std::memory_order_relaxed);
  int f_s = frc.s.load(std::memory_order_relaxed), f_ns = frc.ns.load(std::memory_order_relaxed);
  GamSpPlan best = {3, 4, 1, 2};
  double bt = 1e30;
  const int nk = K / 32;
  if (f_s > 1 && (f_s > 8 || nk % f_s != 0 || nk / f_s < 4)) f_s = 1;
  if (f_ns == 3 && a_mode != 0) f_ns = 2;
  for (int w = 4; w >= 2; w -= 2) {
    if ((f_nw == 2 || f_nw == 4) && w != f_nw) continue;
    for (int t = (w == 2 ? 3 : 4); t >= 2; --t) {
      if (f_mt >= 2 && f_mt <= 4 && t != f_mt && !(w == 2 && f_mt == 4)) continue;
      for (int S = 1; S <= 8; ++S) {
        if (f_s >= 1 && S != f_s) continue;
        if (S > 1 && (nk % S != 0 || nk / S < 4)) continue;
        if (f_s < 1 && S > 1 && (long)gam_cdiv(M, 64 * t) * gam_cdiv(N, 64 * w) * 2 > ncu) continue;
        for (int ns = 2; ns <= 3; ++ns) {
          if (ns == 3 && (!gam_sp_has_ns3(t, w) || a_mode != 0)) continue;
          if ((f_ns == 2 || f_ns == 3) && ns != f_ns && !(f_ns == 3 && !gam_sp_has_ns3(t, w))) continue;
          const double us = gam_gemm_sp_model(M, N, K, a_mode, t, w, S, ncu, ns);
          if (us < bt - 1e-9) { bt = us; best = {t, w, S, ns}; }
        }
      }
    }
  }
  return best;
}

static inline hipError_t gam_launch_gemm_sp(const GamGemmArgs& a_in, int act, hipStream_t stream) {
  GamGemmArgs a = a_in;
  if (a.M <= 0 || a.N <= 0) return hipSuccess;
  if (a.K <= 0 || a.K % 32 != 0 || a.Asp == nullptr || a.Wsp == nullptr) return hipErrorInvalidValue;
  if (a.a_mode == 0 ? (a.lda % 32 != 0) : (a.conv_c % 32 != 0)) return hipErrorInvalidValue;
  if (!gam_gemm_sp_epilogue_ok(a)) return hipErrorInvalidValue;
  int mt = a.sp_mt, nw = a.sp_nw, ns = a.sp_ns;
  if (mt < 2 || mt > 4 || (nw != 2 && nw != 4) || (nw == 2 && mt == 4)) {
    const GamSpPlan p = gam_gemm_sp_plan(a.M, a.N, a.K, a.a_mode);
    mt = p.mt; nw = p.nw; ns = p.ns;
    if (a.splitk > 1 && a.partial == nullptr) return hipErrorInvalidValue;
  }
  if (ns != 3 || !gam_sp_has_ns3(mt, nw)) ns = 2;
  if (a.splitk > 1 && (a.partial == nullptr || (a.K / 32) % a.splitk != 0)) return hipErrorInvalidValue;
  if (a.n_switch > 0 && (a.Asp2 == nullptr || a.a_mode != 0 || a.n_switch % (64 * nw) != 0)) return hipErrorInvalidValue;
  if (a.splitk <= 1) { a.splitk = 0; a.partial = nullptr; }
  const int grid = gam_cdiv(a.M, 64 * mt) * gam_cdiv(a.N, 64 * nw);
  a.ntiles = grid;
#if GAM_SP_INSTRUMENT
  static long long* tl_dev = nullptr;
  static int tl_cap = 0;
  static const bool tl_on = getenv("GAM_SP_TLOG") != nullptr;
  a.tlog = nullptr;
  if (tl_on) {
    if (grid > tl_cap) { if (tl_dev) (void)hipFree(tl_dev); (void)hipMalloc(&tl_dev, (size_t)grid * 64); tl_cap = grid; }
    (void)hipMemsetAsync(tl_dev, 0, (size_t)grid * 64, stream);
    a.tlog = tl_dev;
  }
#endif
#define GAM_LSP(ACTV, EPIV)                                                            \
  if (ns == 3) {                                                                       \
    if (nw == 4) gam_launch_gemm_sp_t<ACTV, EPIV, 2, 4, 3>(a, grid, stream);           \
    else if (mt == 2) gam_launch_gemm_sp_t<ACTV, EPIV, 2, 2, 3>(a, grid, stream);      \
    else gam_launch_gemm_sp_t<ACTV, EPIV, 3, 2, 3>(a, grid, stream);                   \
  } else if (nw == 2) switch (mt) {                                                    \
    case 2: gam_launch_gemm_sp_t<ACTV, EPIV, 2, 2>(a, grid, stream); break;            \
    default: gam_launch_gemm_sp_t<ACTV, EPIV, 3, 2>(a, grid, stream); break;           \
  } else switch (mt) {                                                                 \
    case 2: gam_launch_gemm_sp_t<ACTV, EPIV, 2, 4>(a, grid, stream); break;            \
    case 3: gam_launch_gemm_sp_t<ACTV, EPIV, 3, 4>(a, grid, stream); break;            \
    default: gam_launch_gemm_sp_t<ACTV, EPIV, 4, 4>(a, grid, stream); break;           \
  }
#define GAM_LSP_H16(ACTV)                                                              \
  if (ns == 3) {                                                                       \
    if (nw == 4) gam_launch_gemm_sp_t<ACTV, GAM_EPI_GENERIC, 2, 4, 3, true>(a, grid, stream);      \
    else if (mt == 2) gam_launch_gemm_sp_t<ACTV, GAM_EPI_GENERIC, 2, 2, 3, true>(a, grid, stream); \
    else gam_launch_gemm_sp_t<ACTV, GAM_EPI_GENERIC, 3, 2, 3, true>(a, grid, stream);  \
  } else if (nw == 2) {                                                                \
    if (mt == 2) gam_launch_gemm_sp_t<ACTV, GAM_EPI_GENERIC, 2, 2, 2, true>(a, grid, stream);      \
    else gam_launch_gemm_sp_t<ACTV, GAM_EPI_GENERIC, 3, 2, 2, true>(a, grid, stream);  \
  } else switch (mt) {                                                                 \
    case 2: gam_launch_gemm_sp_t<ACTV, GAM_EPI_GENERIC, 2, 4, 2, true>(a, grid, stream); break;    \
    case 3: gam_launch_gemm_sp_t<ACTV, GAM_EPI_GENERIC, 3, 4, 2, true>(a, grid, stream); break;    \
    default: gam_launch_gemm_sp_t<ACTV, GAM_EPI_GENERIC, 4, 4, 2, true>(a, grid, stream); break;   \
  }
  const int epi = gam_sp_epi_bits(a);
  const int act_k = epi == GAM_EPI_PART ? GAM_ACT_NONE : act;
  enum : int { E_PLAIN = 0, E_RES = GAM_EPI_RESID, E_RESA = GAM_EPI_RESID | GAM_EPI_ALPHA, E_GRD = GAM_EPI_GUARD,
               E_UP = GAM_EPI_SP32 | GAM_EPI_GUARD, E_STEM = GAM_EPI_SP32 | GAM_EPI_GUARD | GAM_EPI_ROWS };
  if (a.h16) {
    switch (act) {
      case GAM_ACT_SILU: GAM_LSP_H16(GAM_ACT_SILU); break;
      case GAM_ACT_RELU: GAM_LSP_H16(GAM_ACT_RELU); break;
      default: GAM_LSP_H16(GAM_ACT_NONE); break;
    }
  } else if (act_k == GAM_ACT_NONE && epi == E_PLAIN) { GAM_LSP(GAM_ACT_NONE, E_PLAIN);
  } else if (act_k == GAM_ACT_NONE && epi == E_RES) { GAM_LSP(GAM_ACT_NONE, E_RES);
  } else if (act_k == GAM_ACT_NONE && epi == E_RESA) { GAM_LSP(GAM_ACT_NONE, E_RESA);
  } else if (act_k == GAM_ACT_NONE && epi == E_GRD) { GAM_LSP(GAM_ACT_NONE, E_GRD);
  } else if (act_k == GAM_ACT_SILU && epi == E_UP) { GAM_LSP(GAM_ACT_SILU, E_UP);
  } else if (act_k == GAM_ACT_RELU && epi == E_STEM) { GAM_LSP(GAM_ACT_RELU, E_STEM);
  } else if (epi == GAM_EPI_PART) { GAM_LSP(GAM_ACT_NONE, GAM_EPI_PART);
  } else {
    switch (act) {
      case GAM_ACT_SILU: GAM_LSP(GAM_ACT_SILU, GAM_EPI_GENERIC); break;
      case GAM_ACT_RELU: GAM_LSP(GAM_ACT_RELU, GAM_EPI_GENERIC); break;
      default: GAM_LSP(GAM_ACT_NONE, GAM_EPI_GENERIC); break;
    }
  }
#undef GAM_LSP
#undef GAM_LSP_H16
#if GAM_SP_INSTRUMENT
  if (tl_on) {
    std::vector<long long> t((size_t)grid * 8);
    (void)hipStreamSynchronize(stream);
    (void)hipMemcpy(t.data(), tl_dev, t.size() * 8, hipMemcpyDeviceToHost);
    long long t_first = t[0], t_last = 0;
    for (int i = 0; i < grid; ++i) { t_first = std::min(t_first, t[i * 8]); t_last = std::max(t_last, t[i * 8 + 3]); }
    auto stat = [&](auto f, const char* name) {
      std::vector<double> v(grid);
      for (int i = 0; i < grid; ++i) v[i] = f(i);
      std::sort(v.begin(), v.end());
      fprintf(stderr, "    %-26s min %7.2f  p50 %7.2f  p90 %7.2f  max %7.2f us\n", name, v[0], v[grid / 2], v[(size_t)(grid * 0.9)], v[grid - 1]);
    };
    fprintf(stderr, "[tlog] M=%d N=%d K=%d MT=%d NW=%d tiles=%d: first entry -> last exit %.2f us\n", a.M, a.N, a.K, mt, nw, grid, (t_last - t_first) * 0.01);
    stat([&](int i) { return (t[i * 8] - t_first) * 0.01; }, "entry after first entry");
    stat([&](int i) { return (t[i * 8 + 1] - t[i * 8]) * 0.01; }, "prologue (2 k-tiles land)");
    stat([&](int i) { return (t[i * 8 + 2] - t[i * 8 + 1]) * 0.01; }, "main loop");
    stat([&](int i) { return (t[i * 8 + 2] - t[i * 8 + 1]) * 0.01 / (a.K / 32); }, "  per k-tile");
    stat([&](int i) { return (double)(t[i * 8 + 6] - t[i * 8 + 5]) / std::max<long long>(1, t[i * 8 + 2] - t[i * 8 + 1]) * 100.0; }, "  shader MHz in loop");
    stat([&](int i) { return (t[i * 8 + 3] - t[i * 8 + 2]) * 0.01; }, "epilogue");
    stat([&](int i) { return (t_last - t[i * 8 + 3]) * 0.01; }, "idle after exit");
    double x_loop[8] = {0}; int x_n[8] = {0};
    for (int i = 0; i < grid; ++i) { const int x = (int)(t[i * 8 + 7] & 7); x_loop[x] += (t[i * 8 + 2] - t[i * 8 + 1]) * 0.01; ++x_n[x]; }
    fprintf(stderr, "    mean loop us by XCD:");
    for (int x = 0; x < 8; ++x) fprintf(stderr, " %.1f", x_n[x] ? x_loop[x] / x_n[x] : 0.0);
    fprintf(stderr, "\n");
  }
#endif
  return hipGetLastError();
}

__global__ __launch_bounds__(256) void gam_to_sp32_kernel(const float* __restrict__ x, _Float16* __restrict__ y,
                                                          size_t n4, const float* __restrict__ rs, int K) {
  const size_t stride = (size_t)gridDim.x * 256;
  for (size_t i = (size_t)blockIdx.x * 256 + threadIdx.x; i < n4; i += stride) {
    f32x4 v = reinterpret_cast<const f32x4*>(x)[i];
    const size_t e = i * 4;
    if (rs != nullptr) v = v * (1.0f / rs[e / (size_t)K]);
    gam_half4 h, l;
    gam_split4(v, h, l);
    _Float16* p = y + (e >> 5) * 64 + (e & 31);
    *reinterpret_cast<gam_half4*>(p) = h;
    *reinterpret_cast<gam_half4*>(p + 32) = l;
  }
}

__global__ __launch_bounds__(256) void gam_to_h16_kernel(const float* __restrict__ x, _Float16* __restrict__ y, size_t n4,
                                                         const float* __restrict__ rs, int K) {
  const size_t stride = (size_t)gridDim.x * 256;
  for (size_t i = (size_t)blockIdx.x * 256 + threadIdx.x; i < n4; i += stride) {
    f32x4 v = reinterpret_cast<const f32x4*>(x)[i];
    if (rs != nullptr) v = v * (1.0f / rs[(i * 4) / (size_t)K]);
    reinterpret_cast<gam_half4*>(y)[i] = __builtin_convertvector(v, gam_half4);
  }
}

__global__ __launch_bounds__(256) void gam_rowscale_kernel(const float* __restrict__ x, float* __restrict__ rs, int rows,
                                                           int K, long lda) {
  const int row = blockIdx.x * 4 + (threadIdx.x >> 6), lane = threadIdx.x & 63;
  if (row >= rows) return;
  const float* xr = x + (size_t)row * lda;
  float m = 0.f;
  for (int k = lane; k < K; k += 64) m = fmaxf(m, fabsf(xr[k]));
  m = gam_wave_max(m);
  float s_, inv_;
  gam_row_scale(m, s_, inv_);
  if (lane == 0) rs[row] = inv_;
}
```

### include/gigaam_hip.h

```cpp
#ifndef GIGAAM_HIP_H
#define GIGAAM_HIP_H

#include <stdint.h>

#ifdef __cplusplus
extern "C" {
#endif

#define GAM_ABI_VERSION 1

typedef struct gam_handle gam_handle;

enum { GAM_SUBS_CONV2D = 0, GAM_SUBS_CONV1D = 1 };
enum { GAM_ATT_ROTARY = 0, GAM_ATT_REL_POS = 1 };
enum { GAM_NORM_BATCH = 0, GAM_NORM_LAYER = 1 };
enum { GAM_HEAD_NONE = 0, GAM_HEAD_CTC = 1, GAM_HEAD_RNNT = 2, GAM_HEAD_EMO = 3 };
enum { GAM_DTYPE_F32 = 0, GAM_DTYPE_F16 = 1, GAM_DTYPE_BF16 = 2, GAM_DTYPE_F64 = 3, GAM_DTYPE_I64 = 4 };

typedef struct gam_config {
  int32_t sample_rate, n_mels, hop_length, win_length, n_fft, center;
  int32_t feat_in, n_layers, d_model, subsampling, subs_kernel_size, subsampling_factor;
  int32_t ff_expansion_factor, self_attention_model, n_heads, pos_emb_max_len;
  int32_t conv_norm_type, conv_kernel_size;
  int32_t head_type, num_classes, pred_hidden, pred_rnn_layers, joint_hidden;
// ... 50 lines not shown
                       float* score, float* loglik, int32_t* status, void* stream);
int gam_op_ctc_align_star(gam_handle* h, const float* log_probs, const int32_t* enc_len, int B, int64_t Tp, int V, const float* star_lp,
                          const int32_t* targets, const int32_t* target_len, int Umax, int32_t* frame_labels, int32_t* tok_first,
                          int32_t* tok_last, float* score, float* loglik, int32_t* status, void* stream);
int gam_op_ctc_align_long_star(gam_handle* h, const float* log_probs, int64_t T, int V, const float* star_lp, const int32_t* targets, int U,
                               int32_t* frame_labels, int32_t* tok_first, int32_t* tok_last, double* score, double* loglik,
                               int32_t* status, void* stream);

int gam_op_ctc_stitch(gam_handle* h, const float* log_probs, const int32_t* enc_len, int B, int64_t Tp, int V, const int32_t* lo,
                      const int32_t* hi, const int64_t* dst, float* out, int64_t T_total, int32_t* status, void* stream);
int gam_op_ctc_greedy_long(gam_handle* h, const float* log_probs, int64_t T, int V, int32_t* ids, int32_t* frames, int32_t* count,
                           void* stream);

int gam_ctc_kws(gam_handle* h, const float* encoded, const int32_t* enc_len, int B, int64_t Tp, int max_hits, int32_t* hit_frames,
                float* hit_score, int32_t* n_hits, float* dense_score, int32_t* dense_start, void* stream);
int gam_op_ctc_kws(gam_handle* h, const float* log_probs, const int32_t* enc_len, int B, int64_t Tp, int V, int max_hits,
                   int32_t* hit_frames, float* hit_score, int32_t* n_hits, float* dense_score, int32_t* dense_start, void* stream);
#define GAM_KWS_STREAM_BEGIN 1
#define GAM_KWS_STREAM_END 2
int64_t gam_ctc_kws_state_bytes(gam_handle* h);
int gam_op_ctc_kws_stream(gam_handle* h, const float* log_probs, int64_t n, int V, int64_t t_base, int flags, void* state, int max_hits,
                          int32_t* hit_frames, float* hit_score, int32_t* n_hits, int32_t* status, float* dense_score,
                          int32_t* dense_start, void* stream);
int gam_set_keywords(gam_handle* h, const int32_t* tokens, const int32_t* offsets, int n_keywords, const float* min_score);

int gam_ctc_beam(gam_handle* h, const float* encoded, const int32_t* enc_len, int B, int64_t Tp, int W, int32_t* ids, int32_t* frames,
                 int32_t* counts, float* score, float* logp, void* stream);
int gam_op_ctc_beam(gam_handle* h, const float* log_probs, const int32_t* enc_len, int B, int64_t Tp, int V, int W, int32_t* ids,
                    int32_t* frames, int32_t* counts, float* score, float* logp, void* stream);
#define GAM_BEAM_STREAM_BEGIN 1
#define GAM_BEAM_STREAM_END 2
int64_t gam_ctc_beam_stream_bytes(gam_handle* h, int W, int64_t max_frames);
int gam_op_ctc_beam_stream(gam_handle* h, const float* log_probs, int64_t n, int V, int64_t t_base, int flags, int W, void* state,
                           int64_t state_bytes, int32_t* ids, int32_t* frames, int32_t* count, double* score, double* logp,
                           int32_t* status, void* stream);
int gam_ctc_beam_nbest(gam_handle* h, const float* encoded, const int32_t* enc_len, int B, int64_t Tp, int W, int N, int32_t* ids,
                       int32_t* frames, int32_t* counts, float* score, float* logp, int32_t* n_hyp, void* stream);
int gam_op_ctc_beam_nbest(gam_handle* h, const float* log_probs, const int32_t* enc_len, int B, int64_t Tp, int V, int W, int N,
                          int32_t* ids, int32_t* frames, int32_t* counts, float* score, float* logp, int32_t* n_hyp, void* stream);
int gam_set_hotwords(gam_handle* h, const int32_t* tokens, const int32_t* offsets, int n_phrases, float boost);
int gam_set_lm(gam_handle* h, const int32_t* token_class, int V, const void* word_table, int64_t word_slots, int word_probe,
               const void* ngram_table, int64_t ngram_slots, int ngram_probe, int order, int bos, int eos, int unk, float unk_logp,
               float weight, float word_bonus);

int gam_rnnt_greedy(gam_handle* h, const float* encoded, const int32_t* enc_len, int B, int64_t Tp,
                    int max_symbols, int32_t* ids, int32_t* frames, int32_t* counts,
                    float* logits_dump, int32_t* dump_count, int dump_cap, void* stream);
int gam_rnnt_encp(gam_handle* h, const float* encoded, int B, int64_t Tp, float* encp_out, void* stream);
int gam_op_rnnt_greedy(gam_handle* h, const float* encp, const int32_t* enc_len, int B, int64_t Tp, int max_symbols, int32_t* ids,
                       int32_t* frames, int32_t* counts, void* stream);
#define GAM_RNNT_STREAM_BEGIN 1
#define GAM_RNNT_STREAM_END 2
int64_t gam_rnnt_greedy_stream_bytes(gam_handle* h);
int gam_op_rnnt_greedy_stream(gam_handle* h, const float* encp, int64_t n, int64_t t_base, int flags, int max_symbols, void* state,
                              int64_t state_bytes, int32_t* ids, int32_t* frames, int64_t cap, int32_t* count, int32_t* status,
                              void* stream);

int gam_rnnt_beam(gam_handle* h, const float* encoded, const int32_t* enc_len, int B, int64_t Tp, int W, int max_symbols, int32_t* ids,
                  int32_t* frames, int32_t* counts, float* score, float* logp, void* stream);
int gam_op_rnnt_beam(gam_handle* h, const float* encp, const int32_t* enc_len, int B, int64_t Tp, int W, int max_symbols, int32_t* ids,
                     int32_t* frames, int32_t* counts, float* score, float* logp, void* stream);

int gam_rnnt_beam_nbest(gam_handle* h, const float* encoded, const int32_t* enc_len, int B, int64_t Tp, int W, int max_symbols, int N,
                        int32_t* ids, int32_t* frames, int32_t* counts, float* score, float* logp, int32_t* n_hyp, void* stream);
int gam_op_rnnt_beam_nbest(gam_handle* h, const float* encp, const int32_t* enc_len, int B, int64_t Tp, int W, int max_symbols, int N,
                           int32_t* ids, int32_t* frames, int32_t* counts, float* score, float* logp, int32_t* n_hyp, void* stream);

int gam_rnnt_align(gam_handle* h, const float* encoded, const int32_t* enc_len, int B, int64_t Tp, const int32_t* targets,
                   const int32_t* target_len, int Umax, int32_t* tok_frame, float* score, float* loglik, int32_t* status, void* stream);
int gam_op_rnnt_align(gam_handle* h, const float* encp, const int32_t* enc_len, int B, int64_t Tp, const int32_t* targets,
                      const int32_t* target_len, int Umax, int32_t* tok_frame, float* score, float* loglik, int32_t* status,
                      float* lattice_out, void* stream);
int gam_op_rnnt_lattice_align(gam_handle* h, const float* lattice, const int32_t* enc_len, int B, int64_t Tp, int V, const int32_t* targets,
                              const int32_t* target_len, int Umax, int32_t* tok_frame, float* score, float* loglik, int32_t* status,
                              void* stream);
int gam_set_rnnt_align_workspace(gam_handle* h, int64_t bytes);

int gam_ctc_confidence(gam_handle* h, const float* encoded, const int32_t* enc_len, int B, int64_t Tp, const int32_t* ids,
                       const int32_t* frames, const int32_t* counts, int cap, int measure, int agg, float* conf, int32_t* span,
                       int32_t* status, void* stream);
int gam_op_ctc_confidence(gam_handle* h, const float* log_probs, const int32_t* enc_len, int B, int64_t Tp, int V, const int32_t* ids,
                          const int32_t* frames, const int32_t* counts, int cap, int measure, int agg, float* conf, int32_t* span,
                          int32_t* status, void* stream);
int gam_op_ctc_confidence_long(gam_handle* h, const float* log_probs, int64_t T, int V, const int32_t* ids, const int32_t* frames,
                               const int32_t* count, int cap, int measure, int agg, int wildcard, float* conf, int32_t* span,
                               int32_t* status, void* stream);
int gam_rnnt_confidence(gam_handle* h, const float* encoded, const int32_t* enc_len, int B, int64_t Tp, const int32_t* ids,
                        const int32_t* frames, const int32_t* counts, int cap, int measure, float* conf, int32_t* status, void* stream);
int gam_op_rnnt_confidence(gam_handle* h, const float* encp, const int32_t* enc_len, int B, int64_t Tp, const int32_t* ids,
                           const int32_t* frames, const int32_t* counts, int cap, int measure, float* conf, int32_t* status, void* stream);

int gam_set_rnnt_cluster(gam_handle* h, int workgroups_per_utterance);
int gam_get_rnnt_cluster(gam_handle* h);
int gam_rnnt_cluster_plan_info(int ncu, int cluster, int exclusive, int B, int H, int JH, int V, int L, int32_t* out);
int gam_rnnt_last_decode(gam_handle* h, int32_t* out);

int gam_debug_buffer_hash(gam_handle* h, int which, uint64_t* hash_out, int64_t* floats_out);

int gam_rnnt_predict(gam_handle* h, const int32_t* labels, const float* h_in, const float* c_in, int B, float* g_out,
                     float* h_out, float* c_out, void* stream);
int gam_rnnt_joint(gam_handle* h, const float* enc, const float* dec, int B, int T, int U, float* log_probs, void* stream);

int gam_emo_probs(gam_handle* h, const float* encoded, const int32_t* enc_len, int B, int64_t Tp, float* probs,
                  void* stream);

enum { GAM_GEMM_F32 = 0, GAM_GEMM_F16X3 = 1, GAM_GEMM_F16 = 2 };
int gam_set_gemm_mode(gam_handle* h, int mode);
int gam_range_flag(gam_handle* h, int* flag_host, void* stream);
int gam_range_flag_fetch(gam_handle* h, int32_t* flag_dev, void* stream);
int gam_get_gemm_mode(const gam_handle* h);

int gam_op_gemm(gam_handle* h, const float* A, const float* W, const float* bias, float* C,
                int M, int N, int K, int act, void* stream);
int gam_op_gemm_ex(gam_handle* h, const float* A, const float* W, const float* bias, const float* R, float alpha,
                   float* C, int M, int N, int K, int act, void* stream);
int gam_op_gemm_fmt(gam_handle* h, const float* A, const float* W, const float* bias, const float* R, float alpha,
                    float* C, int64_t ldc, int M, int N, int K, int act, int c_split, int c_guard, void* stream);

int gam_op_attention(gam_handle* h, const float* q, const float* k, const float* v, float* ctx,
                     const int32_t* lens, int B, int T, int H, void* stream);
int gam_op_attention_ex(gam_handle* h, const float* q, const float* k, const float* v, int64_t ldq, float* ctx,
                        const int32_t* lens, const int32_t* cu, int B, int Ta, int Tv, int H, const float* pbuf,
                        const float* pos_u, const float* pos_v, void* stream);

typedef struct gam_ln_op {
  const float* x;
  float* out1;
  float* out2;
  const float* w1;
  const float* b1;
  const float* w2;
  const float* b2;
  const float* rcos;
  const float* rsin;
  const int32_t* row_t;
  float* rs;
  const float* part;
  const float* pbias;
  const float* presid;
  float* xstore;
  int32_t mode, rows, d, split1, split2, dk, ta, rope_rows, nsplit;
  float eps, palpha;
} gam_ln_op;
int gam_op_layernorm(gam_handle* h, const gam_ln_op* op, void* stream);

int gam_op_convmod(gam_handle* h, const float* u, float* z, const float* dw_w, const float* dw_b, const float* n_scale,
                   const float* n_shift, const int32_t* lens, const int32_t* cu, int B, int Ta, int Tv, int d, int ks,
                   int layer_norm, int z_split, void* stream);

int gam_tune_sp(int mt, int nw, int splitk);
int gam_plan_sp(int M, int N, int K, int n_cu, int* mt, int* nw, int* splitk);
int gam_plan_sp_ex(int M, int N, int K, int n_cu, int* mt, int* nw, int* splitk, int* stages);
int gam_tune_sp_stages(int stages);

enum { GAM_RS_FMT_U8 = 0, GAM_RS_FMT_I16 = 1, GAM_RS_FMT_I24 = 2, GAM_RS_FMT_I32 = 3, GAM_RS_FMT_F32 = 4, GAM_RS_FMT_MULAW = 5,
       GAM_RS_FMT_ALAW = 6 };
int gam_resample_plan(int rate_in, int rate_out, int* up, int* down, int* taps);
int gam_resample_tile(int rate_in, int rate_out, int* tile, int* form);
int gam_resample_table(int rate_in, int rate_out, float* coeff, int32_t* first);
int64_t gam_resample_out_len(int rate_in, int rate_out, int64_t n_in);
int gam_op_resample(const void* src, int fmt, int channels, int channel, const int64_t* len_in, int B, int64_t frames, int rate_in,
                    int rate_out, const float* coeff, const int32_t* first, float* dst, int64_t L_out, int64_t* len_out, void* stream);

enum { GAM_PF_GEMM = 0, GAM_PF_CONV2 = 1, GAM_PF_ATTN = 2, GAM_PF_NORM = 3, GAM_PF_CONVMOD = 4,
       GAM_PF_STEM = 5, GAM_PF_FRONTEND = 6, GAM_PF_DECODE = 7, GAM_PF_MISC = 8,
       GAM_PF_ALIGN_BT = 9, GAM_PF_ALIGN_OUT = 10,
       GAM_PF_NCLASS = 11 };
int gam_profile_enable(gam_handle* h, int on);
int gam_profile_read(gam_handle* h, int cls, double* ms, int64_t* launches, double* work);
int gam_profile_pause(gam_handle* h, int on);
int gam_profile_read_bytes(gam_handle* h, int cls, double* bytes);

typedef struct gam_comm gam_comm;
#define GAM_COMM_ID_BYTES 128
int gam_comm_unique_id(char id_out[GAM_COMM_ID_BYTES]);
int gam_comm_create(const char id[GAM_COMM_ID_BYTES], int rank, int world, int device_id, gam_comm** out);
int gam_comm_world(const gam_comm* c);
int gam_gather_ids(gam_comm* c, const int32_t* index, const int32_t* counts, const int32_t* ids, const int32_t* frames,
                   int rows, int cap, int32_t* all_index, int32_t* all_counts, int32_t* all_ids, int32_t* all_frames,
                   void* stream);
const char* gam_comm_last_error(const gam_comm* c);
void gam_comm_destroy(gam_comm* c);

const char* gam_last_error(const gam_handle* h);

#ifdef __cplusplus
}
#endif
#endif
```

Before: 21320.

## Add persistent resident-tile variant of split-fp16 GEMM overlapping next tile's DMA with epilogue

Adds a RES template variant of the split-fp16 GEMM kernel in which a grid of at most one workgroup per CU loops over output tiles, issuing the next tile's prologue loads before running the current tile's epilogue. The planner turns this on automatically when the tile count is large relative to the CU count, with a tuning knob to force or disable it, and the graph-cache key now includes the force words. The goal is to hide the per-tile prologue latency and launch/tail cost behind the epilogue. In exchange it adds register pressure and serialises tiles within a workgroup, which can hurt load balance.

```diff
diff --git a/gigaam_amd/_lib.py b/gigaam_amd/_lib.py
--- a/gigaam_amd/_lib.py
+++ b/gigaam_amd/_lib.py
@@ -120,6 +120,9 @@
     "gam_plan_sp": (C.c_int, [C.c_int, C.c_int, C.c_int, C.c_int, C.POINTER(C.c_int), C.POINTER(C.c_int), C.POINTER(C.c_int)]),
     "gam_plan_sp_ex": (C.c_int, [C.c_int, C.c_int, C.c_int, C.c_int, C.POINTER(C.c_int), C.POINTER(C.c_int), C.POINTER(C.c_int), C.POINTER(C.c_int)]),
     "gam_tune_sp_stages": (C.c_int, [C.c_int]),
+    "gam_tune_sp_resident": (C.c_int, [C.c_int, C.c_int]),
+    "gam_plan_sp_resident": (C.c_int, [C.c_int, C.c_int, C.c_int, C.c_int, C.c_int]),
+    "gam_tune_sp_words": (C.c_int, [C.POINTER(C.c_int), C.c_int]),
     "gam_resample_plan": (C.c_int, [C.c_int, C.c_int, C.POINTER(C.c_int), C.POINTER(C.c_int), C.POINTER(C.c_int)]),
     "gam_resample_tile": (C.c_int, [C.c_int, C.c_int, C.POINTER(C.c_int), C.POINTER(C.c_int)]),
     "gam_resample_table": (C.c_int, [C.c_int, C.c_int, _P, _P]),
diff --git a/gigaam_amd/csrc/gam_api.hip b/gigaam_amd/csrc/gam_api.hip
--- a/gigaam_amd/csrc/gam_api.hip
+++ b/gigaam_amd/csrc/gam_api.hip
@@ -391,7 +391,7 @@
     }
     GamSpPlan plan = gam_gemm_sp_plan(a.M, a.N, a.K, a.a_mode, h->ncu);
     if (!h->use_splitk) plan.s = 1;
-    a.sp_mt = plan.mt; a.sp_nw = plan.nw; a.sp_ns = plan.ns;
+    a.sp_mt = plan.mt; a.sp_nw = plan.nw; a.sp_ns = plan.ns; a.sp_res = plan.res;
     GamGemmArgs full = a;
     if (plan.s > 1) {
       if (int r = ensure(h, h->splitk_ws, (size_t)plan.s * a.M * a.N + 64)) return r;
@@ -1321,8 +1321,10 @@
   const EncPlan& p = c.p;
   *replayed = false;
   if (!p.graph) return 0;
-  const GamSpForce& frc = gam_sp_force();
-  const std::vector<int> key = {p.B, p.Ta, p.Tv, p.nl, h->gemm_mode, (int)p.sp, h->use_splitk, h->fuse_reduce, frc.mt.load(), frc.nw.load(), frc.s.load(), frc.ns.load()};
+  std::vector<int> key = {p.B, p.Ta, p.Tv, p.nl, h->gemm_mode, (int)p.sp, h->use_splitk, h->fuse_reduce};
+  int forced[GAM_SP_FORCE_WORDS];
+  gam_sp_force_words(forced);
+  key.insert(key.end(), forced, forced + GAM_SP_FORCE_WORDS);
   Entry& ge = h->graphs[key];
   if (ge.gen != h->ws_generation) {
     if (ge.exec) { hipGraphExecDestroy(ge.exec); --h->graph_count; }
@@ -2956,6 +2958,25 @@
   return 0;
 }
 
+int gam_tune_sp_resident(int mode, int grid) {
+  if (mode < -1 || mode > 1 || grid < 0 || grid > 65535) return -1;
+  gam_sp_force().res = mode;
+  gam_sp_force().res_grid = grid;
+  return 0;
+}
+
+int gam_tune_sp_words(int* words, int cap) {
+  int w[GAM_SP_FORCE_WORDS];
+  gam_sp_force_words(w);
+  for (int i = 0; words != nullptr && i < cap && i < GAM_SP_FORCE_WORDS; ++i) words[i] = w[i];
+  return GAM_SP_FORCE_WORDS;
+}
+
+int gam_plan_sp_resident(int M, int N, int K, int n_cu, int conv) {
+  if (M <= 0 || N <= 0 || K <= 0 || K % 32 != 0) return -1;
+  return gam_gemm_sp_plan(M, N, K, conv ? 1 : 0, n_cu > 0 ? n_cu : 256).res;
+}
+
 int gam_plan_sp_ex(int M, int N, int K, int n_cu, int* mt, int* nw, int* splitk, int* stages) {
   if (M <= 0 || N <= 0 || K <= 0 || K % 32 != 0 || !mt || !nw || !splitk || !stages) return -1;
   const GamSpPlan p = gam_gemm_sp_plan(M, N, K, 0, n_cu > 0 ? n_cu : 256);
diff --git a/gigaam_amd/csrc/gam_gemm.h b/gigaam_amd/csrc/gam_gemm.h
--- a/gigaam_amd/csrc/gam_gemm.h
+++ b/gigaam_amd/csrc/gam_gemm.h
@@ -36,6 +36,7 @@
   const float* a_rs;
   int* range_flag;
   int c_guard;
+  int sp_res;
   long long* tlog;
 };
 
diff --git a/gigaam_amd/csrc/gam_gemm_sp.h b/gigaam_amd/csrc/gam_gemm_sp.h
--- a/gigaam_amd/csrc/gam_gemm_sp.h
+++ b/gigaam_amd/csrc/gam_gemm_sp.h
@@ -10,14 +10,14 @@
 #define GAM_SP_INSTRUMENT 0
 #endif
 #if GAM_SP_INSTRUMENT
-#define GAM_SP_TL(i)                                                                  \
+#define GAM_SP_TL(i, T)                                                               \
   if (g.tlog != nullptr && threadIdx.x == 0) {                                        \
-    g.tlog[(size_t)lid * 8 + (i)] = wall_clock64();                                   \
-    if ((i) == 1 || (i) == 2) g.tlog[(size_t)lid * 8 + 4 + (i)] = clock64();          \
-    if ((i) == 0) g.tlog[(size_t)lid * 8 + 7] = blockIdx.x;                            \
+    g.tlog[(size_t)(T) * 8 + (i)] = wall_clock64();                                   \
+    if ((i) == 1 || (i) == 2) g.tlog[(size_t)(T) * 8 + 4 + (i)] = clock64();          \
+    if ((i) == 0) g.tlog[(size_t)(T) * 8 + 7] = (long long)blockIdx.x | ((long long)t_seq << 32);  \
   }
 #else
-#define GAM_SP_TL(i)
+#define GAM_SP_TL(i, T)
 #endif
 
 template <int MT, int NW, int NS = 2>
@@ -49,7 +49,7 @@
   GAM_EPI_GENERIC = 256
 };
 
-template <int ACT, int EPI, int MT, int NW, int NS = 2, bool H16 = false>
+template <int ACT, int EPI, int MT, int NW, int NS = 2, bool H16 = false, bool RES = false>
 __global__ __launch_bounds__(128 * NW, NW == 2 ? 2 : 1) void gam_gemm_sp_kernel(GamGemmArgs g) {
   extern __shared__ __attribute__((aligned(16))) unsigned char gam_smem_sp[];
   using Cfg = GamGemmSpCfg<MT, NW, NS>;
@@ -63,24 +63,52 @@
   const int wm = wave / NW, wn = wave % NW;
 
   const int nbn = (g.N + BN - 1) / BN;
-  const int total = gridDim.x;
-  const int q8 = total >> 3, r8 = total & 7;
   const int bid = blockIdx.x;
-  const int xcd = bid & 7;
-  const int lid = (xcd < r8 ? xcd * (q8 + 1) : r8 * (q8 + 1) + (xcd - r8) * q8) + (bid >> 3);
-  int tm = lid / nbn, tn = lid % nbn;
-  if (g.skip_pad) {
-    tm = bid / nbn;
-    tn = bid % nbn;
-  }
-  const int m0 = tm * BM;
-  const int n0 = tn * BN;
-  if (g.skip_pad && g.lens != nullptr) {
-    const int mlast = m0 + BM - 1 < g.M ? m0 + BM - 1 : g.M - 1;
-    const int b0 = m0 / g.rpb;
-    if (b0 == mlast / g.rpb && (m0 - b0 * g.rpb) / g.fdiv >= g.lens[b0]) return;
-  }
-  GAM_SP_TL(0);
+  int t_cur = 0, t_step = 1, t_end = 1;
+  int t_seq = 0;
+  (void)t_step; (void)t_end; (void)t_seq;
+  int m0, n0;
+  auto tile_is_pad = [&](int pm0) -> bool {
+    if (!(g.skip_pad && g.lens != nullptr)) return false;
+    const int mlast = pm0 + BM - 1 < g.M ? pm0 + BM - 1 : g.M - 1;
+    const int b0 = pm0 / g.rpb;
+    return b0 == mlast / g.rpb && (pm0 - b0 * g.rpb) / g.fdiv >= g.lens[b0];
+  };
+  if constexpr (!RES) {
+    const int total = gridDim.x;
+    const int q8 = total >> 3, r8 = total & 7;
+    const int xcd = bid & 7;
+    const int lid = (xcd < r8 ? xcd * (q8 + 1) : r8 * (q8 + 1) + (xcd - r8) * q8) + (bid >> 3);
+    int tm = lid / nbn, tn = lid % nbn;
+    if (g.skip_pad) {
+      tm = bid / nbn;
+      tn = bid % nbn;
+    }
+    m0 = tm * BM;
+    n0 = tn * BN;
+    if (g.skip_pad && g.lens != nullptr) {
+      const int mlast = m0 + BM - 1 < g.M ? m0 + BM - 1 : g.M - 1;
+      const int b0 = m0 / g.rpb;
+      if (b0 == mlast / g.rpb && (m0 - b0 * g.rpb) / g.fdiv >= g.lens[b0]) return;
+    }
+    t_cur = lid;
+  } else {
+    const int total = g.ntiles, ng = gridDim.x;
+    const bool one_run = ng < 8;
+    const int q8 = one_run ? total : total >> 3, r8 = one_run ? 0 : total & 7;
+    const int xcd = one_run ? 0 : bid & 7;
+    const int xwg = one_run ? bid : bid >> 3;
+    const int t_first = xcd < r8 ? xcd * (q8 + 1) : r8 * (q8 + 1) + (xcd - r8) * q8;
+    t_cur = t_first + xwg;
+    t_step = one_run ? ng : (ng >> 3) + (xcd < (ng & 7) ? 1 : 0);
+    t_end = t_first + q8 + (xcd < r8 ? 1 : 0);
+    if (g.skip_pad) { t_cur = bid; t_step = ng; t_end = total; }
+    while (t_cur < t_end && tile_is_pad((t_cur / nbn) * BM)) t_cur += t_step;
+    if (t_cur >= t_end) return;
+    m0 = (t_cur / nbn) * BM;
+    n0 = (t_cur % nbn) * BN;
+  }
+  GAM_SP_TL(0, t_cur);
 
   auto a_row_off = [&](int m) -> size_t {
     m = m < g.M ? m : g.M - 1;
@@ -88,24 +116,27 @@
     const int fr = m / g.conv_f2, ff = m - fr * g.conv_f2;
     return ((size_t)fr * 2 * g.conv_fp + 2 * ff) * (size_t)g.conv_c;
   };
-  const size_t a_tile0 = a_row_off(m0);
-  const unsigned char* Ab = reinterpret_cast<const unsigned char*>(g.n_switch > 0 && n0 >= g.n_switch ? g.Asp2 : g.Asp) + a_tile0 * 4;
-  const unsigned char* Wb = reinterpret_cast<const unsigned char*>(g.Wsp) + (size_t)n0 * (size_t)g.K * 4;
+  size_t a_tile0;
+  const unsigned char* Ab;
+  const unsigned char* Wb;
   unsigned a_src[NAI], w_src[NWI];
-#pragma unroll
-  for (int i = 0; i < NAI; ++i) {
-    const int row = 8 * (wave + NWAVES * i) + (lane >> 3);
-    const int slot = (lane & 7) ^ gam_sp_key(row);
-    a_src[i] = (unsigned)((a_row_off(m0 + row) - a_tile0) * 4) + slot * 16;
-  }
-#pragma unroll
-  for (int i = 0; i < NWI; ++i) {
-    const int row = 8 * (wave + NWAVES * i) + (lane >> 3);
-    const int slot = (lane & 7) ^ gam_sp_key(row);
-    int n = n0 + row;
-    n = n < g.N ? n : g.N - 1;
-    w_src[i] = (unsigned)(n - n0) * (unsigned)g.K * 4u + slot * 16;
-  }
+#define GAM_SP_SET_TILE(LN)                                                                                      \
+  a_tile0 = a_row_off(m0);                                                                                       \
+  Ab = reinterpret_cast<const unsigned char*>(g.n_switch > 0 && n0 >= g.n_switch ? g.Asp2 : g.Asp) + a_tile0 * 4; \
+  Wb = reinterpret_cast<const unsigned char*>(g.Wsp) + (size_t)n0 * (size_t)g.K * 4;                             \
+  _Pragma("unroll") for (int i = 0; i < NAI; ++i) {                                                              \
+    const int row = 8 * (wave + NWAVES * i) + ((LN) >> 3);                                                       \
+    const int slot = ((LN) & 7) ^ gam_sp_key(row);                                                               \
+    a_src[i] = (unsigned)((a_row_off(m0 + row) - a_tile0) * 4) + slot * 16;                                      \
+  }                                                                                                              \
+  _Pragma("unroll") for (int i = 0; i < NWI; ++i) {                                                              \
+    const int row = 8 * (wave + NWAVES * i) + ((LN) >> 3);                                                       \
+    const int slot = ((LN) & 7) ^ gam_sp_key(row);                                                               \
+    int n = n0 + row;                                                                                            \
+    n = n < g.N ? n : g.N - 1;                                                                                   \
+    w_src[i] = (unsigned)(n - n0) * (unsigned)g.K * 4u + slot * 16;                                              \
+  }
+  GAM_SP_SET_TILE(lane);
 
   f32x4 acc[2 * MT][4];
 #pragma unroll
@@ -123,6 +154,8 @@
     const int cb = kt_first / 9, t9 = kt_first - cb * 9;
     d_c0 = 32 * cb; d_kh = t9 / 3; d_kw = t9 - d_kh * 3;
   }
+  const int d_c0_first = d_c0, d_kw_first = d_kw, d_kh_first = d_kh;
+  (void)d_c0_first; (void)d_kw_first; (void)d_kh_first;
   auto dma_ka = [&]() -> size_t {
     if (g.a_mode == 0) return (size_t)d_kt * 128;
     return (((size_t)d_kh * g.conv_fp + d_kw) * (size_t)g.conv_c + d_c0) * 4;
@@ -136,29 +169,39 @@
       if (++d_kh == 3) { d_kh = 0; d_c0 += 32; }
     }
   };
+#define GAM_SP_UNIFORM(PA, PW) \
+  if constexpr (RES) { asm volatile("" : "+s"(PA)); asm volatile("" : "+s"(PW)); }
   auto issue = [&](int stage) {
     unsigned char* sb = gam_smem_sp + stage * Cfg::STAGE + wave * 1024;
     const unsigned char* ab = Ab + dma_ka();
     const unsigned char* wb = Wb + (size_t)d_kt * 128;
-#pragma unroll
-    for (int i = 0; i < NAI; ++i)
-      __builtin_amdgcn_global_load_lds((glb_ptr_t)(ab + a_src[i]), (lds_ptr_t)(sb + i * (NWAVES * 1024)), 16, 0, 0);
-#pragma unroll
-    for (int i = 0; i < NWI; ++i)
-      __builtin_amdgcn_global_load_lds((glb_ptr_t)(wb + w_src[i]), (lds_ptr_t)(sb + Cfg::A_BYTES + i * (NWAVES * 1024)), 16, 0, 0);
+    GAM_SP_UNIFORM(ab, wb);
+#pragma unroll
+    for (int i = 0; i < NAI; ++i) {
+      unsigned off_ = a_src[i];
+      if constexpr (RES) asm volatile("" : "+v"(off_));
+      __builtin_amdgcn_global_load_lds((glb_ptr_t)(ab + off_), (lds_ptr_t)(sb + i * (NWAVES * 1024)), 16, 0, 0);
+    }
+#pragma unroll
+    for (int i = 0; i < NWI; ++i) {
+      unsigned off_ = w_src[i];
+      if constexpr (RES) asm volatile("" : "+v"(off_));
+      __builtin_amdgcn_global_load_lds((glb_ptr_t)(wb + off_), (lds_ptr_t)(sb + Cfg::A_BYTES + i * (NWAVES * 1024)), 16, 0, 0);
+    }
     dma_advance();
   };
 
-  const int fi = lane & 15, fg = lane >> 4;
-  const int wr = 8 * (fi >> 2) + (fi & 3);
   int o_a[2][2], o_w[2][2];
-#pragma unroll
-  for (int pl = 0; pl < 2; ++pl)
-#pragma unroll
-    for (int x = 0; x < 2; ++x) {
-      o_a[pl][x] = fi * 128 + (((4 * pl + fg) ^ gam_sp_key(fi + 16 * x)) << 4);
-      o_w[pl][x] = (wr + 4 * x) * 128 + (((4 * pl + fg) ^ gam_sp_key(wr + 4 * x)) << 4);
-    }
+#define GAM_SP_FRAG_OFFS(LN)                                                                      \
+  {                                                                                               \
+    const int fi = (LN) & 15, fg = (LN) >> 4;                                                     \
+    const int wr = 8 * (fi >> 2) + (fi & 3);                                                      \
+    _Pragma("unroll") for (int pl = 0; pl < 2; ++pl) _Pragma("unroll") for (int x = 0; x < 2; ++x) {  \
+      o_a[pl][x] = fi * 128 + (((4 * pl + fg) ^ gam_sp_key(fi + 16 * x)) << 4);                   \
+      o_w[pl][x] = (wr + 4 * x) * 128 + (((4 * pl + fg) ^ gam_sp_key(wr + 4 * x)) << 4);          \
+    }                                                                                             \
+  }
+  GAM_SP_FRAG_OFFS(lane);
   const int a_base = wm * (BM / 2) * 128;
   const int w_base = Cfg::A_BYTES + wn * 64 * 128;
 
@@ -205,6 +248,7 @@
   auto half1 = [&](const unsigned char* sn, int istage) {
     const unsigned char* ab = Ab + dma_ka();
     const unsigned char* wb = Wb + (size_t)d_kt * 128;
+    GAM_SP_UNIFORM(ab, wb);
     unsigned char* sb = gam_smem_sp + istage * Cfg::STAGE + wave * 1024;
     dma_advance();
 #pragma unroll
@@ -218,10 +262,12 @@
       }
       const int gi = u < QM ? u - 2 * MT : (u - QM < 4 ? -1 : G3 + u - QM - 4);
       if (gi >= 0 && gi < NG) {
+        unsigned off_ = gi < NAI ? a_src[gi % NAI] : w_src[(gi - NAI + NWI) % NWI];
+        if constexpr (RES) asm volatile("" : "+v"(off_));
         if (gi < NAI)
-          __builtin_amdgcn_global_load_lds((glb_ptr_t)(ab + a_src[gi % NAI]), (lds_ptr_t)(sb + gi * (NWAVES * 1024)), 16, 0, 0);
+          __builtin_amdgcn_global_load_lds((glb_ptr_t)(ab + off_), (lds_ptr_t)(sb + gi * (NWAVES * 1024)), 16, 0, 0);
         else
-          __builtin_amdgcn_global_load_lds((glb_ptr_t)(wb + w_src[(gi - NAI + NWI) % NWI]),
+          __builtin_amdgcn_global_load_lds((glb_ptr_t)(wb + off_),
                                            (lds_ptr_t)(sb + Cfg::A_BYTES + (gi - NAI) * (NWAVES * 1024)), 16, 0, 0);
       }
       __builtin_amdgcn_sched_barrier(0);
@@ -232,13 +278,15 @@
   static_assert(VMW < 64, "vmcnt field");
 #pragma unroll
   for (int st_ = 0; st_ < NS; ++st_) issue(st_);
+  GAM_SP_TL(4, t_cur);
+  for (;;) {
   if constexpr (NS == 2) {
     __builtin_amdgcn_s_waitcnt(0x0070);
     __syncthreads();
   } else {
     asm volatile("s_waitcnt vmcnt(%0) lgkmcnt(0)\n\ts_barrier" ::"n"(VMW) : "memory");
   }
-  GAM_SP_TL(1);
+  GAM_SP_TL(1, t_cur);
 #pragma unroll
   for (int q = 0; q < 2 * MT; ++q) GAM_SP_RDA(0, q, gam_smem_sp);
 #pragma unroll
@@ -262,8 +310,9 @@
 #undef GAM_SP_RDW
 #undef GAM_SP_RDA
 #undef GAM_SP_MFMA
+#undef GAM_SP_UNIFORM
   __builtin_amdgcn_s_waitcnt(0x0070);
-  GAM_SP_TL(2);
+  GAM_SP_TL(2, t_cur);
 
   const int mw = m0 + wm * (BM / 2), nw = n0 + wn * 64;
 
@@ -275,7 +324,9 @@
   const bool need_bt = !part && (GEN ? (g.lens != nullptr || g.remap) : (EPI & GAM_EPI_ROWS) != 0);
   const bool guard = GEN ? (g.c_guard && g.range_flag != nullptr) : (EPI & GAM_EPI_GUARD) != 0;
   const bool tail = GEN ? (g.N & 4) != 0 : (EPI & GAM_EPI_TAIL) != 0;
-  const int lrow = lane & 15, lq8 = (lane >> 4) * 8;
+  int lane_e = lane;
+  if constexpr (RES) asm volatile("" : "+v"(lane_e));
+  const int lrow = lane_e & 15, lq8 = (lane_e >> 4) * 8;
   const float accscale = g.wscale_inv;
   const int ecol0 = nw + lq8;
   bool c_ok[2], c_both[2];
@@ -322,6 +373,32 @@
     }
     r_rsc[i] = accscale * ((ok && g.a_rs != nullptr) ? g.a_rs[row] : 1.0f);
     r_ok[i] = ok; r_masked[i] = masked; r_orow[i] = orow;
+  }
+  int t_nxt = t_end;
+  if constexpr (RES) {
+    t_nxt = t_cur + t_step;
+    while (t_nxt < t_end && tile_is_pad((t_nxt / nbn) * BM)) t_nxt += t_step;
+    if (t_nxt < t_end) {
+#pragma unroll
+      for (int pp = 0; pp < 2; ++pp)
+#pragma unroll
+        for (int hf = 0; hf < 2; ++hf) asm volatile("" : "+v"(bv[pp][hf]));
+#pragma unroll
+      for (int i = 0; i < 2 * MT; ++i) asm volatile("" : "+v"(r_rsc[i]));
+      __builtin_amdgcn_s_waitcnt(0x0070);
+      __syncthreads();
+      ++t_seq;
+      GAM_SP_TL(0, t_nxt);
+      m0 = (t_nxt / nbn) * BM;
+      n0 = (t_nxt % nbn) * BN;
+      int lane_s = lane;
+      asm volatile("" : "+v"(lane_s));
+      GAM_SP_SET_TILE(lane_s);
+      d_kt = kt_first; d_c0 = d_c0_first; d_kw = d_kw_first; d_kh = d_kh_first;
+#pragma unroll
+      for (int st_ = 0; st_ < NS; ++st_) issue(st_);
+      GAM_SP_TL(4, t_nxt);
+    }
   }
   if (part) {
 #pragma unroll
@@ -406,8 +483,25 @@
 #undef GAM_SP_LDR
 #if GAM_SP_INSTRUMENT
   if (g.tlog != nullptr) { __builtin_amdgcn_s_waitcnt(0x0070); __syncthreads(); }
-  GAM_SP_TL(3);
+  GAM_SP_TL(3, t_cur);
 #endif
+  if (!RES || t_nxt >= t_end) break;
+  t_cur = t_nxt;
+  {
+    int lane_n = lane;
+    asm volatile("" : "+v"(lane_n));
+    GAM_SP_SET_TILE(lane_n);
+    GAM_SP_FRAG_OFFS(lane_n);
+  }
+#pragma unroll
+  for (int i = 0; i < 2 * MT; ++i)
+#pragma unroll
+    for (int j = 0; j < 4; ++j)
+#pragma unroll
+      for (int r = 0; r < 4; ++r) acc[i][j][r] = 0.f;
+  }
+#undef GAM_SP_SET_TILE
+#undef GAM_SP_FRAG_OFFS
 }
 
 static inline bool gam_gemm_sp_epilogue_ok(const GamGemmArgs& a) {
@@ -416,12 +510,13 @@
          (a.R == nullptr || (a.ldr % 4 == 0 && al16(a.R)));
 }
 
-template <int ACT, int EPI, int MT, int NW, int NS = 2, bool H16 = false>
+template <int ACT, int EPI, int MT, int NW, int NS = 2, bool H16 = false, bool RES = false>
 static inline void gam_launch_gemm_sp_t(const GamGemmArgs& a, int grid, hipStream_t stream) {
   static std::atomic<unsigned long long> attr_devs{0};
   constexpr int smem = GamGemmSpCfg<MT, NW, NS>::SMEM;
   static_assert(smem <= 160 * 1024, "LDS stages do not fit a CU");
-  auto kern = gam_gemm_sp_kernel<ACT, EPI, MT, NW, NS, H16>;
+  static_assert(!RES || (NW == 4 && NS == 2 && !H16), "resident form: the 8-wave two-stage tiles (one workgroup per CU)");
+  auto kern = gam_gemm_sp_kernel<ACT, EPI, MT, NW, NS, H16, RES>;
   if (gam_set_max_lds(reinterpret_cast<const void*>(kern), smem, attr_devs) != hipSuccess) return;
   hipLaunchKernelGGL(kern, dim3(grid, a.splitk > 1 ? a.splitk : 1), dim3(128 * NW), smem, stream, a);
 }
@@ -433,10 +528,12 @@
          ((a.N & 7) == 4 ? GAM_EPI_TAIL : 0);
 }
 
-struct GamSpPlan { int mt, nw, s, ns; };
+struct GamSpPlan { int mt, nw, s, ns, res; };
 struct GamSpForce {
-  std::atomic<int> mt{0}, nw{0}, s{0}, ns{0};
+  std::atomic<int> mt{0}, nw{0}, s{0}, ns{0}, res{-1}, res_grid{0};
   GamSpForce() {
+    const char* e4 = getenv("GAM_SP_PERSIST");
+    res = e4 ? (atoi(e4) != 0 ? 1 : 0) : -1;
     const char* e0 = getenv("GAM_SP_MT"); const char* e1 = getenv("GAM_SP_NW"); const char* e2 = getenv("GAM_SP_SPLITK");
     const char* e3 = getenv("GAM_SP_STAGES");
     mt = e0 ? atoi(e0) : 0; nw = e1 ? atoi(e1) : 0; s = e2 ? atoi(e2) : 0; ns = e3 ? atoi(e3) : 0;
@@ -444,6 +541,11 @@
 };
 static inline bool gam_sp_has_ns3(int mt, int nw) { return (nw == 2 && (mt == 2 || mt == 3)) || (nw == 4 && mt == 2); }
 static inline GamSpForce& gam_sp_force() { static GamSpForce f; return f; }
+#define GAM_SP_FORCE_WORDS 6
+static inline void gam_sp_force_words(int* w) {
+  const GamSpForce& f = gam_sp_force();
+  w[0] = f.mt.load(); w[1] = f.nw.load(); w[2] = f.s.load(); w[3] = f.ns.load(); w[4] = f.res.load(); w[5] = f.res_grid.load();
+}
 static inline double gam_gemm_sp_model(int M, int N, int K, int a_mode, int t, int w, int S, int ncu, int ns = 2) {
   const long wgs = (long)gam_cdiv(M, 64 * t) * gam_cdiv(N, 64 * w) * S;
   const int nkt = K / 32 / S;
@@ -475,11 +577,20 @@
   if (S > 1) us += 7.1 + (double)(S + 2) * M * N * 4.0 / 3.87e6;
   return us;
 }
+static inline bool gam_sp_has_resident(int mt, int nw, int ns) { return nw == 4 && ns == 2 && (mt == 3 || mt == 4); }
+static inline int gam_sp_resident_grid(long tiles, int nk, int mt, int nw, int S, int ns, int ncu) {
+  GamSpForce& frc = gam_sp_force();
+  const int f_res = frc.res.load(std::memory_order_relaxed), f_grid = frc.res_grid.load(std::memory_order_relaxed);
+  if (f_res == 0 || S > 1 || !gam_sp_has_resident(mt, nw, ns) || tiles <= 0) return 0;
+  if (f_res < 0 && (nk > 96 ? tiles < 4L * ncu : tiles * 5 <= (long)ncu * 6)) return 0;
+  if (f_grid > 0) return f_grid;
+  return (int)(tiles < ncu ? tiles : ncu);
+}
 static inline GamSpPlan gam_gemm_sp_plan(int M, int N, int K, int a_mode = 0, int ncu = 256) {
   GamSpForce& frc = gam_sp_force();
   const int f_mt = frc.mt.load(std::memory_order_relaxed), f_nw = frc.nw.load(std::memory_order_relaxed);
   int f_s = frc.s.load(std::memory_order_relaxed), f_ns = frc.ns.load(std::memory_order_relaxed);
-  GamSpPlan best = {3, 4, 1, 2};
+  GamSpPlan best = {3, 4, 1, 2, 0};
   double bt = 1e30;
   const int nk = K / 32;
   if (f_s > 1 && (f_s > 8 || nk % f_s != 0 || nk / f_s < 4)) f_s = 1;
@@ -496,11 +607,12 @@
           if (ns == 3 && (!gam_sp_has_ns3(t, w) || a_mode != 0)) continue;
           if ((f_ns == 2 || f_ns == 3) && ns != f_ns && !(f_ns == 3 && !gam_sp_has_ns3(t, w))) continue;
           const double us = gam_gemm_sp_model(M, N, K, a_mode, t, w, S, ncu, ns);
-          if (us < bt - 1e-9) { bt = us; best = {t, w, S, ns}; }
+          if (us < bt - 1e-9) { bt = us; best = {t, w, S, ns, 0}; }
         }
       }
     }
   }
+  best.res = gam_sp_resident_grid((long)gam_cdiv(M, 64 * best.mt) * gam_cdiv(N, 64 * best.nw), nk, best.mt, best.nw, best.s, best.ns, ncu);
   return best;
 }
 
@@ -510,10 +622,10 @@
   if (a.K <= 0 || a.K % 32 != 0 || a.Asp == nullptr || a.Wsp == nullptr) return hipErrorInvalidValue;
   if (a.a_mode == 0 ? (a.lda % 32 != 0) : (a.conv_c % 32 != 0)) return hipErrorInvalidValue;
   if (!gam_gemm_sp_epilogue_ok(a)) return hipErrorInvalidValue;
-  int mt = a.sp_mt, nw = a.sp_nw, ns = a.sp_ns;
+  int mt = a.sp_mt, nw = a.sp_nw, ns = a.sp_ns, res = a.sp_res;
   if (mt < 2 || mt > 4 || (nw != 2 && nw != 4) || (nw == 2 && mt == 4)) {
     const GamSpPlan p = gam_gemm_sp_plan(a.M, a.N, a.K, a.a_mode);
-    mt = p.mt; nw = p.nw; ns = p.ns;
+    mt = p.mt; nw = p.nw; ns = p.ns; res = p.res;
     if (a.splitk > 1 && a.partial == nullptr) return hipErrorInvalidValue;
   }
   if (ns != 3 || !gam_sp_has_ns3(mt, nw)) ns = 2;
@@ -559,6 +671,13 @@
     case 3: gam_launch_gemm_sp_t<ACTV, GAM_EPI_GENERIC, 3, 4, 2, true>(a, grid, stream); break;    \
     default: gam_launch_gemm_sp_t<ACTV, GAM_EPI_GENERIC, 4, 4, 2, true>(a, grid, stream); break;   \
   }
+#define GAM_LSP_RES(ACTV, EPIV)                                                        \
+  launched_res = true;                                                                 \
+  if (mt == 3) gam_launch_gemm_sp_t<ACTV, EPIV, 3, 4, 2, false, true>(a, res, stream); \
+  else gam_launch_gemm_sp_t<ACTV, EPIV, 4, 4, 2, false, true>(a, res, stream);
+  bool launched_res = false;
+  (void)launched_res;
+  const bool resident = res > 0 && a.splitk <= 1 && !a.h16 && gam_sp_has_resident(mt, nw, ns);
   const int epi = gam_sp_epi_bits(a);
   const int act_k = epi == GAM_EPI_PART ? GAM_ACT_NONE : act;
   enum : int { E_PLAIN = 0, E_RES = GAM_EPI_RESID, E_RESA = GAM_EPI_RESID | GAM_EPI_ALPHA, E_GRD = GAM_EPI_GUARD,
@@ -569,6 +688,10 @@
       case GAM_ACT_RELU: GAM_LSP_H16(GAM_ACT_RELU); break;
       default: GAM_LSP_H16(GAM_ACT_NONE); break;
     }
+  } else if (resident && act_k == GAM_ACT_NONE && epi == E_PLAIN) { GAM_LSP_RES(GAM_ACT_NONE, E_PLAIN);
+  } else if (resident && act_k == GAM_ACT_NONE && epi == E_GRD) { GAM_LSP_RES(GAM_ACT_NONE, E_GRD);
+  } else if (resident && act_k == GAM_ACT_SILU && epi == E_UP) { GAM_LSP_RES(GAM_ACT_SILU, E_UP);
+  } else if (resident && act_k == GAM_ACT_RELU && epi == E_STEM) { GAM_LSP_RES(GAM_ACT_RELU, E_STEM);
   } else if (act_k == GAM_ACT_NONE && epi == E_PLAIN) { GAM_LSP(GAM_ACT_NONE, E_PLAIN);
   } else if (act_k == GAM_ACT_NONE && epi == E_RES) { GAM_LSP(GAM_ACT_NONE, E_RES);
   } else if (act_k == GAM_ACT_NONE && epi == E_RESA) { GAM_LSP(GAM_ACT_NONE, E_RESA);
@@ -584,30 +707,46 @@
     }
   }
 #undef GAM_LSP
+#undef GAM_LSP_RES
 #undef GAM_LSP_H16
 #if GAM_SP_INSTRUMENT
   if (tl_on) {
     std::vector<long long> t((size_t)grid * 8);
     (void)hipStreamSynchronize(stream);
     (void)hipMemcpy(t.data(), tl_dev, t.size() * 8, hipMemcpyDeviceToHost);
-    long long t_first = t[0], t_last = 0;
-    for (int i = 0; i < grid; ++i) { t_first = std::min(t_first, t[i * 8]); t_last = std::max(t_last, t[i * 8 + 3]); }
-    auto stat = [&](auto f, const char* name) {
-      std::vector<double> v(grid);
-      for (int i = 0; i < grid; ++i) v[i] = f(i);
+    std::vector<int> ran, prev(grid, -1);
+    for (int i = 0; i < grid; ++i) if (t[i * 8] != 0) ran.push_back(i);
+    if (ran.empty()) return hipGetLastError();
+    {
+      std::vector<int> ord(ran);
+      std::sort(ord.begin(), ord.end(), [&](int a, int b) { return t[a * 8 + 7] < t[b * 8 + 7] ? true : (t[a * 8 + 7] > t[b * 8 + 7] ? false : a < b); });
+      auto wg = [&](int i) { return (long long)(t[i * 8 + 7] & 0xffffffffll); };
+      std::stable_sort(ord.begin(), ord.end(), [&](int a, int b) { return wg(a) < wg(b); });
+      for (size_t j = 1; j < ord.size(); ++j) if (wg(ord[j]) == wg(ord[j - 1])) prev[ord[j]] = ord[j - 1];
+    }
+    long long t_first = t[ran[0] * 8], t_last = 0;
+    for (int i : ran) { t_first = std::min(t_first, t[i * 8]); t_last = std::max(t_last, t[i * 8 + 3]); }
+    auto stat = [&](auto f, const char* name, int which = 0) {
+      std::vector<double> v;
+      for (int i : ran) if (which == 0 || (which == 1) == (prev[i] < 0)) v.push_back(f(i));
+      if (v.empty()) return;
       std::sort(v.begin(), v.end());
-      fprintf(stderr, "    %-26s min %7.2f  p50 %7.2f  p90 %7.2f  max %7.2f us\n", name, v[0], v[grid / 2], v[(size_t)(grid * 0.9)], v[grid - 1]);
+      const size_t n = v.size();
+      fprintf(stderr, "    %-26s min %7.2f  p50 %7.2f  p90 %7.2f  max %7.2f us\n", name, v[0], v[n / 2], v[(size_t)(n * 0.9)], v[n - 1]);
     };
-    fprintf(stderr, "[tlog] M=%d N=%d K=%d MT=%d NW=%d tiles=%d: first entry -> last exit %.2f us\n", a.M, a.N, a.K, mt, nw, grid, (t_last - t_first) * 0.01);
-    stat([&](int i) { return (t[i * 8] - t_first) * 0.01; }, "entry after first entry");
-    stat([&](int i) { return (t[i * 8 + 1] - t[i * 8]) * 0.01; }, "prologue (2 k-tiles land)");
+    fprintf(stderr, "[tlog] M=%d N=%d K=%d MT=%d NW=%d tiles=%d: first entry -> last exit %.2f us (%s, %d workgroups, %d tiles ran)\n", a.M, a.N, a.K,
+            mt, nw, grid, (t_last - t_first) * 0.01, launched_res ? "resident" : "one tile per workgroup", launched_res ? res : grid, (int)ran.size());
+    stat([&](int i) { return (t[i * 8] - t_first) * 0.01; }, "entry after first entry", 1);
+    stat([&](int i) { return (t[i * 8 + 1] - t[i * 8]) * 0.01; }, "prologue (2 k-tiles land)", 1);
     stat([&](int i) { return (t[i * 8 + 2] - t[i * 8 + 1]) * 0.01; }, "main loop");
     stat([&](int i) { return (t[i * 8 + 2] - t[i * 8 + 1]) * 0.01 / (a.K / 32); }, "  per k-tile");
     stat([&](int i) { return (double)(t[i * 8 + 6] - t[i * 8 + 5]) / std::max<long long>(1, t[i * 8 + 2] - t[i * 8 + 1]) * 100.0; }, "  shader MHz in loop");
     stat([&](int i) { return (t[i * 8 + 3] - t[i * 8 + 2]) * 0.01; }, "epilogue");
+    stat([&](int i) { return (t[i * 8 + 4] - t[i * 8 + 2]) * 0.01; }, "seam: loop end -> DMA issued", 2);
+    stat([&](int i) { return (t[i * 8 + 1] - t[prev[i] * 8 + 3]) * 0.01; }, "seam wait: epilogue -> MFMA", 2);
     stat([&](int i) { return (t_last - t[i * 8 + 3]) * 0.01; }, "idle after exit");
     double x_loop[8] = {0}; int x_n[8] = {0};
-    for (int i = 0; i < grid; ++i) { const int x = (int)(t[i * 8 + 7] & 7); x_loop[x] += (t[i * 8 + 2] - t[i * 8 + 1]) * 0.01; ++x_n[x]; }
+    for (int i : ran) { const int x = (int)(t[i * 8 + 7] & 7); x_loop[x] += (t[i * 8 + 2] - t[i * 8 + 1]) * 0.01; ++x_n[x]; }
     fprintf(stderr, "    mean loop us by XCD:");
     for (int x = 0; x < 8; ++x) fprintf(stderr, " %.1f", x_n[x] ? x_loop[x] / x_n[x] : 0.0);
     fprintf(stderr, "\n");
diff --git a/include/gigaam_hip.h b/include/gigaam_hip.h
--- a/include/gigaam_hip.h
+++ b/include/gigaam_hip.h
@@ -226,6 +226,9 @@
 int gam_plan_sp(int M, int N, int K, int n_cu, int* mt, int* nw, int* splitk);
 int gam_plan_sp_ex(int M, int N, int K, int n_cu, int* mt, int* nw, int* splitk, int* stages);
 int gam_tune_sp_stages(int stages);
+int gam_tune_sp_resident(int mode, int grid);
+int gam_plan_sp_resident(int M, int N, int K, int n_cu, int conv);
+int gam_tune_sp_words(int* words, int cap);
 
 enum { GAM_RS_FMT_U8 = 0, GAM_RS_FMT_I16 = 1, GAM_RS_FMT_I24 = 2, GAM_RS_FMT_I32 = 3, GAM_RS_FMT_F32 = 4, GAM_RS_FMT_MULAW = 5,
        GAM_RS_FMT_ALAW = 6 };
```

After: 21360 (median of 5 runs). No clear change (+0.2%).
